# cschin/Peregrine

Hardware: AMD Instinct MI355X
Metric: confirmed overlaps/sec (ovlp_t records, index+overlap stages, seqdb resident in HBM) (higher is better)
Workload: dtype u8/u32 integer

## Files before the change

peregrine_amd/csrc/pgx_replay.h:

```cpp
#pragma once
#include "pgx_internal.h"

namespace pgx {
namespace rp {

constexpr uint32_t NIL = 0;
constexpr uint32_t NONE = 0xFFFFFFFFu;
constexpr int END_FUZZ = 48;
enum { T_OVERLAP = 0, T_CONTAINS = 1, T_CONTAINED = 2 };

constexpr uint32_t NIN = 58;
struct alignas(16) PHot {
  unsigned long long key;
  uint32_t own;
  uint32_t pad;
};
struct alignas(256) PCold {
  uint32_t cnt;
  uint32_t rhead;
  uint32_t in[NIN];
  uint32_t pad[4];
};
static_assert(sizeof(PHot) == 16 && sizeof(PCold) == 256, "pair slot = 16 hot bytes + four cold cache lines");
struct MSlot {
  unsigned long long a;
  uint32_t b;
  uint32_t req;
};
struct Item {
  uint32_t pslot;
  uint32_t info;
  uint32_t mslot;
  uint32_t next;
};
struct RNode {
  uint32_t next, bucket;
};
constexpr uint32_t I_GUESS = 1u << 18, I_UNFILED = 1u << 19;
#ifndef PGX_SPARSE_CAP
#define PGX_SPARSE_CAP 65536
#endif
constexpr uint32_t SPARSE_CAP = PGX_SPARSE_CAP;
constexpr uint32_t LIST_CAP = 262144;
constexpr uint32_t DEV_LIST = 0xFFFFFFFFu, DEV_LIST_WIN = 0xFFFFFFFEu;
enum : uint32_t { OV_ITEMS = 1, OV_NODES = 2, OV_REQS = 4, OV_PAIRS = 8, OV_MEMO = 16, OV_QOFF = 32, OV_PASSES = 64 };
constexpr uint8_t F_DUP = 1, F_GUESS = 2, F_UNFILED = 4;
constexpr uint8_t F_BIG = 8;

struct alignas(64) Counters {
  uint32_t item_top, rnode_top, nreq, overflow;
  uint32_t pad0[12];
  uint32_t ndirty, min_dirty, max_dirty, pad;
  uint32_t nbig;
  uint32_t nbig_total;
  uint32_t pad1[10];
  unsigned long long lookups, skips, evals, records;
#ifdef PGX_BIG_STATS
  uint32_t big_max_steps, big_long, big_long_n, big_evals;
  unsigned long long pad2[2];
#else
  unsigned long long pad2[4];
#endif
};

struct R {
  uint32_t nb;
  const uint32_t *bid, *bstart;
  const uint64_t *y0;
  const uint8_t *dir;
  const uint32_t *rlen;
  PHot *ph;
  PCold *pc;
  uint32_t cshift;
  uint32_t pmask;
  MSlot *mt;
  uint32_t mmask;
  Item *items;
  uint32_t item_cap;
  RNode *rn;
  uint32_t rn_cap;
  pgx_align_key *rq_key;
  pgx_match *rq_res;
  uint32_t req_cap, settled;
  uint32_t memo_used;
  uint8_t *dirty, *evaluated, *parity, *bflags, *ever;
  uint32_t *ihead, *inum, *ohead, *lookups, *skips;
  uint32_t *dlist;
  uint32_t *blist;
  uint32_t wlist0;
  uint4 *wcur;
  Counters *c;
  unsigned long long *spread;
  uint32_t bestn;
  uint32_t tail;
  int predict, predict2;
  uint32_t big_min;
  uint32_t dup_min;
  uint32_t wbig0;
};

__device__ __forceinline__ uint64_t mix64(uint64_t h) {
  h ^= h >> 33, h *= 0xff51afd7ed558ccdULL, h ^= h >> 33, h *= 0xc4ceb9fe1a85ec53ULL, h ^= h >> 33;
  return h;
}
__device__ __forceinline__ uint32_t own_enc(uint32_t j, uint32_t par, uint32_t type) { return ((j << 3) | (par << 2) | type) + 1; }
__device__ __forceinline__ uint32_t own_bucket(uint32_t v) { return (v - 1) >> 3; }
__device__ __forceinline__ uint32_t own_parity(uint32_t v) { return ((v - 1) >> 2) & 1; }
__device__ __forceinline__ uint32_t own_type(uint32_t v) { return (v - 1) & 3; }
__device__ __forceinline__ uint32_t lane_rank(uint64_t m) {
  return __builtin_amdgcn_mbcnt_hi((uint32_t)(m >> 32), __builtin_amdgcn_mbcnt_lo((uint32_t)m, 0u));
}
__device__ __forceinline__ long iabs64(long x) { return x < 0 ? -x : x; }

__device__ __forceinline__ bool classify(const pgx_match &m, uint32_t rlen0, uint32_t rlen1, uint32_t q_off, uint32_t *type) {
  const uint32_t slen0 = rlen0 - q_off, slen1 = rlen1;
  *type = T_OVERLAP;
  if (m.q_bgn < END_FUZZ && m.t_bgn < END_FUZZ &&
      (iabs64((long)slen0 - m.q_end) < END_FUZZ || iabs64((long)slen1 - m.t_end) < END_FUZZ) && m.q_end > 500 &&
      m.t_end > 500) {
    if (iabs64((long)rlen0 - ((long)m.q_end - m.q_bgn)) < END_FUZZ * 2 ||
        iabs64((long)rlen1 - ((long)m.t_end - m.t_bgn)) < END_FUZZ * 2)
      *type = rlen0 >= rlen1 ? T_CONTAINS : T_CONTAINED;
    return true;
  }
  return false;
}

__device__ __forceinline__ bool predict_contained(uint32_t rlen0, uint32_t rlen1, uint32_t q_off, int mq, int mt) {
  return (int)rlen1 - (int)(rlen0 - q_off) < mt || q_off < (uint32_t)mq;
}

__device__ __forceinline__ uint32_t pair_slot(const R &r, uint64_t pair) {
  const unsigned long long want = pair + 1;
  uint32_t i = (uint32_t)mix64(pair) & r.pmask;
  for (int probes = 0; probes < 1024; ++probes) {
    unsigned long long k = r.ph[i].key;
    if (k == want) return i;
    if (k == 0) {
      k = atomicCAS(&r.ph[i].key, 0ULL, want);
      if (k == 0 || k == want) return i;
    }
    i = (i + 1) & r.pmask;
  }
  atomicOr(&r.c->overflow, OV_PAIRS);
  return i;
}

__device__ __forceinline__ uint32_t pair_find(const R &r, uint64_t pair, uint32_t *own) {
  const unsigned long long want = pair + 1;
  uint32_t i = (uint32_t)mix64(pair) & r.pmask;
  for (int probes = 0; probes < 1024; ++probes) {
    const uint4 h = *reinterpret_cast<const uint4 *>(&r.ph[i]);
    const unsigned long long k = (unsigned long long)h.y << 32 | h.x;
    if (k == want) {
      *own = h.z;
      return i;
    }
    if (k == 0) break;
    i = (i + 1) & r.pmask;
  }
  *own = 0;
  return NONE;
}

__device__ __forceinline__ uint32_t memo_find(const R &r, unsigned long long a, uint32_t b, uint32_t *req) {
  uint32_t i = (uint32_t)mix64(a ^ mix64(b)) & r.mmask;
  for (int probes = 0; probes < 1024; ++probes) {
    const uint4 h = *reinterpret_cast<const uint4 *>(&r.mt[i]);
    const unsigned long long cur = (unsigned long long)h.y << 32 | h.x;
    if (cur == 0) break;
    if (cur == a && h.z == b + 1) {
      *req = h.w;
      return i;
    }
    i = (i + 1) & r.mmask;
  }
  *req = NONE;
  return NONE;
}

struct Ent {
  uint32_t rid, pos1;
};
__device__ __forceinline__ Ent entry_of(uint64_t y) { return Ent{(uint32_t)(y >> 32), (((uint32_t)y) >> 1) + 1}; }

constexpr uint32_t NCH = 256;
constexpr uint32_t SPREAD = 256;
constexpr uint32_t ICH = 128;

#ifndef PGX_REPLAY_GL
#define PGX_REPLAY_GL 16
#endif
constexpr int GL = PGX_REPLAY_GL;
constexpr uint32_t GPW = 64 / GL, GPB = 256 / GL;
__device__ __forceinline__ uint64_t gbits(uint64_t wave_mask, int gbase) { return (wave_mask >> gbase) & ((1ULL << GL) - 1ULL); }

__device__ __forceinline__ uint64_t bucket_of_group(const R &r, uint32_t lo, uint32_t hi, uint32_t nlist, uint32_t g) {
  if (nlist) {
    const uint32_t n = nlist == DEV_LIST ? min(r.c->ndirty, SPARSE_CAP) : nlist == DEV_LIST_WIN ? min(r.c->ndirty, LIST_CAP) : nlist;
    return g < n ? (uint64_t)r.dlist[g] : (uint64_t)hi;
  }
  return (uint64_t)lo + g;
}

__device__ __forceinline__ void mark_readers(const R &r, uint32_t slot, uint32_t j) {
  const uint32_t *w = reinterpret_cast<const uint32_t *>(&r.pc[slot >> r.cshift]);
  const uint4 h1 = *reinterpret_cast<const uint4 *>(w);
  const uint32_t c = min(h1.x, NIN);
  if (c > 0 && h1.z > j + 1 && h1.z <= r.nb) r.dirty[h1.z - 1] = 1;
  if (c > 1 && h1.w > j + 1 && h1.w <= r.nb) r.dirty[h1.w - 1] = 1;
  for (uint32_t q = 2; q < c; q += 8) {
    const uint4 a = *reinterpret_cast<const uint4 *>(w + 2 + q), b = *reinterpret_cast<const uint4 *>(w + 6 + q);
    const uint32_t x[8] = {a.x, a.y, a.z, a.w, b.x, b.y, b.z, b.w};
#pragma unroll
    for (uint32_t k = 0; k < 8; ++k)
      if (q + k < c && x[k] > j + 1 && x[k] <= r.nb) r.dirty[x[k] - 1] = 1;
  }
  if (c < NIN) return;
  for (uint32_t nd = h1.y; nd != NIL; nd = r.rn[nd - 1].next) {
    const uint32_t rb = r.rn[nd - 1].bucket;
    if (rb > j) r.dirty[rb] = 1;
  }
}

struct M128 {
  uint64_t lo, hi;
};
__device__ __forceinline__ int popc128(M128 m) { return __popcll(m.lo) + __popcll(m.hi); }
__device__ __forceinline__ bool any128(M128 m) { return (m.lo | m.hi) != 0; }
__device__ __forceinline__ int ctz128(M128 m) { return m.lo ? __builtin_ctzll(m.lo) : 64 + __builtin_ctzll(m.hi); }
__device__ __forceinline__ int nth128(M128 m, uint32_t nth) {
  const uint32_t cl = (uint32_t)__popcll(m.lo);
  uint64_t w = m.lo;
  int base = 0;
  if (nth > cl) w = m.hi, nth -= cl, base = 64;
  for (uint32_t k = 1; k < nth; ++k) w &= w - 1;
  return base + __builtin_ctzll(w);
}
__device__ __forceinline__ M128 upto128(int stop) {
  M128 m;
  m.lo = stop >= 63 ? ~0ULL : ((2ULL << stop) - 1ULL);
  m.hi = stop < 64 ? 0ULL : (stop >= 127 ? ~0ULL : ((2ULL << (stop - 64)) - 1ULL));
  return m;
}
__device__ __forceinline__ M128 and128(M128 a, M128 b) { return M128{a.lo & b.lo, a.hi & b.hi}; }
__device__ __forceinline__ M128 andn128(M128 a, M128 b) { return M128{a.lo & ~b.lo, a.hi & ~b.hi}; }
__device__ __forceinline__ M128 shr128(M128 m, uint32_t s) {
  if (s >= 128) return M128{0, 0};
  if (s >= 64) return M128{m.hi >> (s - 64), 0};
  if (s == 0) return m;
  return M128{m.lo >> s | m.hi << (64 - s), m.hi >> s};
}




#ifndef PGX_BIG_NW
#define PGX_BIG_NW 8
#endif
constexpr int BIG_NW = PGX_BIG_NW;
constexpr int BIG_NR = BIG_NW / 2;
constexpr uint32_t BIG_WG = 512;
constexpr uint32_t SET_CAP = 2048, CLAIM_CAP = 1024;
constexpr uint32_t CB = 4096;

__global__ void k_setup(R r, uint32_t *hist);
__global__ void k_init_slots(uint4 *__restrict__ wcur, uint32_t nslots, uint32_t n_dense, uint32_t wlist0, Counters *c);
__global__ void k_eval(R r, uint32_t lo, uint32_t hi, uint32_t nlist);
template <int GLT, int PW>
__global__ void k_eval_rows(R r, uint32_t lo, uint32_t hi, uint32_t nlist);
__global__ void k_eval_big(R r, uint32_t lo, uint32_t hi, uint32_t nlist);
__global__ void k_update(R r, uint32_t lo, uint32_t hi, uint32_t nlist);
__global__ void k_count_a(R r, uint32_t rlo, uint32_t rhi, uint32_t *__restrict__ blk);
__global__ void k_count_b(R r, uint32_t rlo, uint32_t rhi, const uint32_t *__restrict__ blk, uint32_t nblk);
__global__ void k_file(R r, uint32_t limit);
__global__ void k_settle(R r);
__global__ void k_emit(R r, const uint32_t *__restrict__ off, pgx_ovlp *__restrict__ out);
__global__ void k_count_pairs(const PHot *__restrict__ ph, uint32_t cap, unsigned long long *__restrict__ out);

}
}
```

peregrine_amd/csrc/pgx_replay.hip:

```cpp
#include <optional>

#include "pgx_replay.h"

namespace pgx {
using namespace rp;
namespace {
uint32_t pow2_at_least(size_t x) {
  size_t c = 1024;
  while (c < x) c <<= 1;
  return (uint32_t)c;
}
unsigned cdiv256(size_t n) { return (unsigned)((n + 255) / 256); }
int env_int(const char *name, int unset) { return getenv(name) ? atoi(getenv(name)) : unset; }
template <typename T>
void alloc_tagged(const char *tag, DevBuf<T> &buf, size_t n) { MemTag t(tag); buf.alloc(n); }

constexpr size_t ITEMS_PER_ENTRY = 6, ITEMS_PER_BUCKET = 64, NODES_PER_ENTRY = 8, REQS_PER_ENTRY = 1;
constexpr size_t STATE_PER_BUCKET = 64;
constexpr double TABLE_LOAD = 0.4;

struct Usage {
  double pairs = 0, reqs = 0, items = 0, nodes = 0;
  void raise(const Usage &u) { pairs = std::max(pairs, u.pairs), reqs = std::max(reqs, u.reqs), items = std::max(items, u.items), nodes = std::max(nodes, u.nodes); }
};
struct Mult {
  double items = 1, nodes = 1, reqs = 1, pairs = 1, memo = 1;
  static Mult from(const Usage &learned, size_t ne, size_t nb) {
    Mult m;
    if (learned.pairs > 0) {
      const double items_default = (double)ITEMS_PER_ENTRY + (double)ITEMS_PER_BUCKET * (double)nb / ne;
      m.items = std::max(0.2, learned.items * 1.25 / items_default), m.nodes = std::max(0.02, learned.nodes * 2 / NODES_PER_ENTRY);
      m.reqs = std::max(1.0, learned.reqs * 1.2);
      m.pairs = std::max(1.0, learned.pairs / TABLE_LOAD), m.memo = std::max(1.0, learned.reqs / TABLE_LOAD);
    }
    if (getenv("PGX_REPLAY_PAIRS_X")) m.pairs = atof(getenv("PGX_REPLAY_PAIRS_X"));
    if (getenv("PGX_REPLAY_MEMO_X")) m.memo = atof(getenv("PGX_REPLAY_MEMO_X"));
    return m;
  }
  void grow(uint32_t ov) {
    auto arena = [](double &m) { m = m < 1 ? 1.0 : m * 2; };
    if (ov & OV_ITEMS) arena(items);
    if (ov & OV_NODES) arena(nodes);
    if (ov & OV_REQS) arena(reqs);
    if (ov & OV_PAIRS) pairs *= 4;
    if (ov & (OV_MEMO | OV_REQS)) memo *= 4;
  }
};

struct Sizes {
  uint32_t pcap, mcap;
  uint32_t cshift = 0;
  size_t ccap = 0;
  uint32_t item_cap, rn_cap, req_cap;
  Sizes(size_t ne, size_t nb, const Mult &m) {
    const size_t top = 0x7FFFFFF0u;
    pcap = pow2_at_least((size_t)(ne * m.pairs)), mcap = pow2_at_least((size_t)(ne * m.memo));
    item_cap = (uint32_t)std::min((size_t)((ne * ITEMS_PER_ENTRY + nb * ITEMS_PER_BUCKET) * m.items) +
                                      (size_t)(nb / GPW + 2 + SPARSE_CAP + 8 + BIG_WG * BIG_NW) * ICH + (1u << 20), top);
    rn_cap = (uint32_t)std::min((size_t)(ne * NODES_PER_ENTRY * m.nodes) + (1u << 20), top);
    req_cap = (uint32_t)std::min((size_t)(ne * REQS_PER_ENTRY * m.reqs) + 65536, top);
  }
  void share_readers(size_t free_bytes) {
    if (getenv("PGX_REPLAY_COLD_SHIFT")) cshift = (uint32_t)std::min(3, std::max(0, env_int("PGX_REPLAY_COLD_SHIFT", 0)));
    else
      while (cshift < 3 && ((size_t)pcap >> cshift) * sizeof(PCold) > free_bytes / 3) ++cshift;
    ccap = ((size_t)pcap >> cshift) + 1;
  }
};
size_t default_need(size_t ne, size_t nb) {
  return (size_t)pow2_at_least(ne) * (sizeof(PHot) + sizeof(PCold) + sizeof(MSlot)) +
         ne * (ITEMS_PER_ENTRY * sizeof(Item) + NODES_PER_ENTRY * sizeof(RNode) + REQS_PER_ENTRY * (sizeof(pgx_align_key) + sizeof(pgx_match))) +
         nb * (ITEMS_PER_BUCKET * sizeof(Item) + STATE_PER_BUCKET) + (256u << 20);
}

struct Tables {
  DevBuf<PHot> hot;
  DevBuf<PCold> cold;
  DevBuf<MSlot> memo;
  bool hot_zero = false, cold_zero = false, memo_zero = false;
  bool held() const { return hot.p != nullptr; }
  size_t bytes() const { return hot.n * sizeof(PHot) + cold.n * sizeof(PCold) + memo.n * sizeof(MSlot); }
  void alloc(size_t pcap, size_t ccap, size_t mcap) {
    if (pcap && hot.n != pcap) alloc_tagged("replay.pair_table_hot", hot, pcap), hot_zero = false;
    if (ccap && cold.n != ccap) alloc_tagged("replay.pair_table_readers", cold, ccap), cold_zero = false;
    if (mcap && memo.n != mcap) alloc_tagged("replay.memo_table", memo, mcap), memo_zero = false;
  }
  void clear(hipStream_t s) {
    if (!hot_zero) PGX_HIP(hipMemsetAsync(hot.p, 0, hot.n * sizeof(PHot), s));
    if (!cold_zero) PGX_HIP(hipMemsetAsync(cold.p, 0, cold.n * sizeof(PCold), s));
    if (!memo_zero) PGX_HIP(hipMemsetAsync(memo.p, 0, memo.n * sizeof(MSlot), s));
    hot_zero = cold_zero = memo_zero = true;
  }
  void drop() { hot.release(), cold.release(), memo.release(), hot_zero = cold_zero = memo_zero = false; }
};
}

struct ReplayState {
  Tables pre;
  size_t last_pcap = 0, last_ccap = 0, last_mcap = 0;
  Usage learned;
  void forget() { pre.drop(), last_pcap = last_ccap = last_mcap = 0, learned = Usage(); }
  Counters *hc = nullptr;
  unsigned long long *hs = nullptr;
  hipStream_t side_stream = nullptr;
  hipEvent_t side_ev[2] = {nullptr, nullptr};
  void handles() {
    if (!hc) PGX_HIP(hipHostMalloc((void **)&hc, sizeof(Counters), hipHostMallocDefault));
    if (!hs) PGX_HIP(hipHostMalloc((void **)&hs, SPREAD * 8 * sizeof(unsigned long long), hipHostMallocDefault));
    if (!side_stream) PGX_HIP(hipStreamCreateWithFlags(&side_stream, hipStreamNonBlocking));
    for (auto &e : side_ev)
      if (!e) PGX_HIP(hipEventCreateWithFlags(&e, hipEventDisableTiming));
  }
  ~ReplayState() {
    if (hc) (void)hipHostFree(hc);
    if (hs) (void)hipHostFree(hs);
    if (side_stream) (void)hipStreamDestroy(side_stream);
    for (auto &e : side_ev)
      if (e) (void)hipEventDestroy(e);
  }
};
void CacheFree::operator()(ReplayState *r) const { delete r; }

namespace {
constexpr size_t WIN0 = 16384, WIN1 = 131072;
constexpr size_t DENSE_DEN = 3;
constexpr size_t TAIL_MAX = 4000;
constexpr uint32_t AHEAD = 24;
constexpr int CHAIN = 8;
constexpr size_t BIG_BATCH = 100000;

enum class Narrow { eval, rows };
struct Walk {
  const pgx_seqdb *const db;
  ReplayState &rs;
  const size_t nb, ne;
  const int band;
  const bool trace;
  const hipStream_t s = ctx().stream;
  const double t0 = wall_ms();
  const bool timed = env_int("PGX_REPLAY_TIMING", 0) != 0;
  const bool deep = env_int("PGX_TRACE", 0) >= 2;
  const size_t window = getenv("PGX_REPLAY_WIN") ? (size_t)atoll(getenv("PGX_REPLAY_WIN")) : (size_t)262144;
  const int inner = env_int("PGX_REPLAY_K", 2);
  Sizes z;
  Tables tab;
  DevBuf<uint32_t> bid, words, dlist, blist, cblk;
  DevBuf<Item> items;
  DevBuf<RNode> rn;
  DevBuf<pgx_align_key> rq_key;
  DevBuf<pgx_match> rq_res;
  DevBuf<uint8_t> bytes;
  DevBuf<uint4> wcur;
  DevBuf<Counters> dc;
  DevBuf<unsigned long long> spread;
  R r;
  Counters *hc = nullptr;
  bool use_big = false;
  size_t n_dirty;
  uint32_t d_lo = 0, d_hi;
  bool known = true;
  bool have_list = false;
  unsigned sweeps = 0, rounds_total = 0;
  size_t first_req = 0;
  size_t first_batch = 0;
  double align_ms = 0;
  Walk(const pgx_seqdb *db_, size_t nb_, size_t ne_, int band_, bool trace_, const Mult &mult)
      : db(db_), rs(get_or_make(db_->caches.replay)), nb(nb_), ne(ne_), band(band_), trace(trace_), z(ne_, nb_, mult), n_dirty(nb_), d_hi((uint32_t)nb_) {
    memset(&r, 0, sizeof(r));
  }
  void alloc_tables() {
    Tables &pre = rs.pre;
    const bool forced = getenv("PGX_REPLAY_COLD_SHIFT") != nullptr;
    const size_t pre_hold = pre.bytes();
    const bool take = pre.held() && pre.hot.n == z.pcap && pre.memo.n == z.mcap && !forced;
    if (take) tab.hot = std::move(pre.hot), tab.memo = std::move(pre.memo), tab.hot_zero = tab.memo_zero = true;
    tab.alloc(z.pcap, 0, 0);
    size_t free_b = 0, total_b = 0;
    const bool measured = !forced && hipMemGetInfo(&free_b, &total_b) == hipSuccess;
    z.share_readers(measured ? free_b + dev_cache_free_bytes() + pre_hold : SIZE_MAX);
    if (take && pre.cold.n == z.ccap) tab.cold = std::move(pre.cold), tab.cold_zero = true;
    else pre.cold.release();
    tab.alloc(z.pcap, z.ccap, z.mcap);
    pre.drop();
    r.ph = tab.hot.p, r.pc = tab.cold.p, r.cshift = z.cshift, r.pmask = z.pcap - 1, r.mt = tab.memo.p, r.mmask = z.mcap - 1;
  }
  void alloc_state() {
    r.item_cap = z.item_cap, r.rn_cap = z.rn_cap, r.req_cap = z.req_cap;
    alloc_tagged("replay.items", items, r.item_cap), alloc_tagged("replay.reader_nodes", rn, r.rn_cap);
    alloc_tagged("replay.requests", rq_key, r.req_cap), alloc_tagged("replay.requests", rq_res, r.req_cap);
    r.items = items.p, r.rn = rn.p, r.rq_key = rq_key.p, r.rq_res = rq_res.p;
    bytes.alloc(nb * 5), words.alloc(nb * 5);
    r.dirty = bytes.p, r.evaluated = bytes.p + nb, r.parity = bytes.p + 2 * nb, r.bflags = bytes.p + 3 * nb, r.ever = bytes.p + 4 * nb;
    r.ihead = words.p, r.inum = words.p + nb, r.ohead = words.p + 2 * nb, r.lookups = words.p + 3 * nb, r.skips = words.p + 4 * nb;
    wcur.alloc(nb + 2 + SPARSE_CAP + 1 + (size_t)BIG_WG * BIG_NW);
    r.wcur = wcur.p, r.wlist0 = (uint32_t)(nb + 2), r.wbig0 = (uint32_t)(nb + 2 + SPARSE_CAP + 1);
    dlist.alloc(LIST_CAP), blist.alloc(LIST_CAP + 64), dc.alloc(1), spread.alloc(SPREAD * 8);
    r.dlist = dlist.p, r.blist = blist.p, r.c = dc.p, r.spread = spread.p;
  }
  void setup(const DevicePairs &dp, const uint32_t *visit_bids, const uint32_t *d_bids, uint32_t bestn) {
    rs.handles(), hc = rs.hc;
    r.nb = (uint32_t)nb;
    if (!d_bids) bid.alloc(nb), bid.upload(visit_bids, nb);
    r.bid = d_bids ? d_bids : bid.p, r.bstart = dp.bstart.p, r.y0 = dp.y0.p, r.dir = dp.dir.p, r.rlen = db->d_rlen.p;
    alloc_tables();
    alloc_state();
    r.big_min = (uint32_t)std::max(0, env_int("PGX_REPLAY_BIG", 48));
    r.dup_min = (uint32_t)std::max(0, env_int("PGX_REPLAY_DUP", 12));
    r.predict = std::max(END_FUZZ * 2 - 8, 1), r.predict2 = END_FUZZ * 2 - 8;
    r.bestn = bestn, r.settled = 0;
    PGX_HIP(hipMemsetAsync(spread.p, 0, SPREAD * 8 * sizeof(unsigned long long), s));
    {
      std::optional<KernelTimer> tm;
      if (timed) tm.emplace("replay_misc", nb);
      const bool took = tab.hot_zero, took_cold = tab.cold_zero;
      tab.clear(s);
      if (trace && took) fprintf(stderr, "[pgx]   replay tables taken over pre-cleared (pair table%s, memo)\n", took_cold ? ", reader lists" : "");
      PGX_HIP(hipMemsetAsync(bytes.p, 0, nb * 5, s));
      PGX_HIP(hipMemsetAsync(words.p, 0, nb * 5 * sizeof(uint32_t), s));
      PGX_HIP(hipMemsetAsync(dc.p, 0, sizeof(Counters), s));
      hipLaunchKernelGGL(k_init_slots, dim3(cdiv256(wcur.n)), dim3(256), 0, s, wcur.p, (uint32_t)wcur.n, (uint32_t)(nb / GPW + 2), r.wlist0, dc.p);
      if (trace) setup_with_histogram();
      else hipLaunchKernelGGL(k_setup, dim3(cdiv256(nb)), dim3(256), 0, s, r, (uint32_t *)nullptr);
    }
    if (r.big_min || r.dup_min) {
      fetch(false);
      use_big = hc->nbig_total != 0;
    }
    cblk.alloc((nb + CB - 1) / CB * 3);
  }
  void setup_with_histogram() {
    DevBuf<uint32_t> hist(32);
    PGX_HIP(hipMemsetAsync(hist.p, 0, 32 * sizeof(uint32_t), s));
    hipLaunchKernelGGL(k_setup, dim3(cdiv256(nb)), dim3(256), 0, s, r, hist.p);
    uint32_t h[32];
    hist.download(h, 32);
    sync();
    fprintf(stderr, "[pgx]   buckets by entries / 8 (last class: >= 120):");
    for (int i = 0; i < 16; ++i) fprintf(stderr, " %u", h[i]);
    fprintf(stderr, "\n[pgx]   ... of those holding a read twice (one partner at a time):");
    for (int i = 0; i < 16; ++i) fprintf(stderr, " %u", h[16 + i]);
    fprintf(stderr, "\n");
  }
  void fetch(bool totals, bool counters = true) {
    if (counters) PGX_HIP(hipMemcpyAsync(hc, dc.p, sizeof(Counters), hipMemcpyDeviceToHost, s));
    if (totals) PGX_HIP(hipMemcpyAsync(rs.hs, spread.p, SPREAD * 8 * sizeof(unsigned long long), hipMemcpyDeviceToHost, s));
    sync();
    if (totals) sum_totals();
  }
  void sum_totals() {
    const unsigned long long *hs = rs.hs;
    hc->evals = hc->lookups = hc->skips = 0;
    hc->records = 0;
    for (uint32_t i = 0; i < SPREAD; ++i) hc->evals += hs[i * 8], hc->lookups += hs[i * 8 + 1], hc->skips += hs[i * 8 + 2], hc->records += hs[i * 8 + 7];
#ifdef PGX_BIG_STATS
    unsigned long long b3 = 0, b4 = 0, b5 = 0, b6 = 0, b7 = 0;
    for (uint32_t i = 0; i < SPREAD; ++i) b3 += hs[i * 8 + 3], b4 += hs[i * 8 + 4], b5 += hs[i * 8 + 5], b6 += hs[i * 8 + 6], b7 += hs[i * 8 + 7];
    fprintf(stderr, "[pgx]   k_eval_big so far: %u evaluations, %llu steps, %llu rows committed; steps cut at a duplicate %llu, ended by a containment %llu, all rows %llu; longest %u steps, %u evaluations of >= 64 steps (entries %u)\n",
            hc->big_evals, b3, b4, b5, b6, b7, hc->big_max_steps, hc->big_long, hc->big_long_n);
#endif
#ifdef PGX_SETTLE_STATS
    unsigned long long c3 = 0, c4 = 0, c5 = 0, c6 = 0;
    for (uint32_t i = 0; i < SPREAD; ++i) c3 += hs[i * 8 + 3], c4 += hs[i * 8 + 4], c5 += hs[i * 8 + 5], c6 += hs[i * 8 + 6];
    fprintf(stderr, "[pgx]   wrong guesses so far: type %llu, rejected short overlap %llu, rejected no match %llu, rejected other %llu\n", c3, c4, c5, c6);
#endif
  }
  void learn_dirty() { n_dirty = hc->ndirty, known = true, d_lo = n_dirty ? hc->min_dirty : 0, d_hi = n_dirty ? hc->max_dirty + 1 : 0; }
  uint32_t gave_up(uint32_t ov) {
    if (trace || !(ov & (OV_ITEMS | OV_NODES | OV_REQS | OV_PAIRS | OV_MEMO)))
      fprintf(stderr, "[pgx] note: the device replay gave up (code %u: items %u of %u, reader nodes %u of %u, requests %u of %u)\n", ov,
              hc->item_top, r.item_cap, hc->rnode_top, r.rn_cap, hc->nreq, r.req_cap);
    return ov;
  }
  void count(uint32_t lo = 0, uint32_t hi = NONE) {
    hi = std::min<uint32_t>(hi, (uint32_t)nb);
    const uint32_t nbl = std::max<uint32_t>(1, (hi - lo + CB - 1) / CB);
    std::optional<KernelTimer> tm;
    if (timed) tm.emplace("replay_misc", 0);
    hipLaunchKernelGGL(k_count_a, dim3(nbl), dim3(256), 0, s, r, lo, hi, cblk.p);
    hipLaunchKernelGGL(k_count_b, dim3(nbl), dim3(256), 0, s, r, lo, hi, cblk.p, nbl);
  }
  void count_all() { count(), have_list = true; }
  void pass(uint32_t lo, uint32_t hi, uint32_t list, Narrow narrow, uint32_t groups, uint64_t units) {
    std::optional<KernelTimer> tm;
    if (timed) tm.emplace(narrow == Narrow::rows ? "replay_rows" : "replay_dense", units);
    const bool walled = deep && list != DEV_LIST;
    double td = 0, t_eval = 0;
    if (walled) sync(), td = wall_ms();
    if (list == DEV_LIST_WIN) count(lo, hi);
    const uint32_t a = list ? 0u : lo, b = list ? (uint32_t)nb : hi;
    const uint32_t big_a = list == DEV_LIST_WIN ? LIST_CAP : list == DEV_LIST ? groups : lo;
    const dim3 big_grid(std::min<uint32_t>(BIG_WG, groups)), big_block(64 * BIG_NW), grid(cdiv256((size_t)groups * GL));
    const bool side = use_big && list && !timed && !deep;
    if (side) {
      PGX_HIP(hipEventRecord(rs.side_ev[0], s));
      PGX_HIP(hipStreamWaitEvent(rs.side_stream, rs.side_ev[0], 0));
      hipLaunchKernelGGL(k_eval_big, big_grid, big_block, 0, rs.side_stream, r, big_a, b, list);
      PGX_HIP(hipEventRecord(rs.side_ev[1], rs.side_stream));
    }
    if (narrow == Narrow::rows) hipLaunchKernelGGL((k_eval_rows<64, 16>), dim3(cdiv256((size_t)groups * 64)), dim3(256), 0, s, r, a, b, list);
    else hipLaunchKernelGGL(k_eval, grid, dim3(256), 0, s, r, a, b, list);
    tm.reset();
    if (side) {
      PGX_HIP(hipStreamWaitEvent(s, rs.side_ev[1], 0));
    } else if (use_big) {
      if (timed) tm.emplace("replay_big", 0);
      hipLaunchKernelGGL(k_eval_big, big_grid, big_block, 0, s, r, big_a, b, list);
      tm.reset();
    }
    if (walled) sync(), t_eval = wall_ms() - td, td = wall_ms();
    if (timed) tm.emplace("replay_update", 0);
    hipLaunchKernelGGL(k_update, grid, dim3(256), 0, s, r, a, b, list);
    tm.reset();
    if (walled) sync(), fprintf(stderr, "[pgx]     iteration: eval %.3f ms, update %.3f ms\n", t_eval, wall_ms() - td);
  }
  void dense_round(bool first_pass) {
    const size_t a_lo = d_lo & ~(size_t)63;
    const size_t win = n_dirty > window / 4 ? window : (size_t)(d_hi - a_lo);
    const size_t cap = first_pass ? std::min(WIN1, win) : win;
    size_t step = first_pass ? std::min(WIN0, cap) : win;
    for (size_t lo = a_lo, nxt; lo < d_hi; lo = nxt, step = std::min(step * 2, cap)) {
      nxt = lo + step;
      const uint32_t hi = (uint32_t)std::min<size_t>(d_hi, nxt), n = hi - (uint32_t)lo;
      for (int k = 0; k < inner; ++k) {
        const bool from_list = !(first_pass && k == 0) && n <= LIST_CAP;
        pass((uint32_t)lo, hi, from_list ? DEV_LIST_WIN : 0u, Narrow::eval, n, k == 0 ? n : 0);
      }
    }
    count_all();
  }
  void sparse_chain() {
    if (!have_list) count_all();
    const size_t est = known && n_dirty <= SPARSE_CAP / 4 ? std::max<size_t>(n_dirty * 4, 1024) : (size_t)SPARSE_CAP;
    const uint32_t groups = (uint32_t)std::min<size_t>(est, SPARSE_CAP);
    for (int c = 0; c < CHAIN; ++c) {
      pass(0, (uint32_t)nb, DEV_LIST, Narrow::rows, groups, 0);
      count_all();
    }
  }
  uint32_t file_and_fetch(unsigned rounds) {
    {
      std::optional<KernelTimer> tm;
      if (timed) tm.emplace("replay_misc", 0);
      hipLaunchKernelGGL(k_file, dim3(cdiv256(nb)), dim3(256), 0, s, r, (uint32_t)nb);
    }
    fetch(trace);
    if (hc->overflow) return hc->overflow;
    learn_dirty();
    r.memo_used = hc->nreq != 0;
    if (trace)
      fprintf(stderr, "[pgx]   round %u: %zu dirty left in [%u, %u), %llu evaluations, t = +%.2f ms\n", rounds, n_dirty, d_lo, d_hi,
              (unsigned long long)hc->evals, wall_ms() - t0);
    return 0;
  }
  uint32_t align_and_settle(size_t nreq) {
    const double a0 = wall_ms();
    const size_t batch = nreq - first_req;
    if (sweeps == 1) first_batch = batch;
    r.tail = batch <= std::max(TAIL_MAX, first_batch / 256) ? AHEAD : 0u;
    dev_align(db, r.rq_key + first_req, batch, band, r.rq_res + first_req, sweeps > 2 ? 2 : sweeps > 1 ? 1 : 0);
    r.settled = (uint32_t)nreq, first_req = nreq;
    {
      std::optional<KernelTimer> tm;
      if (timed) tm.emplace("replay_misc", 0);
      hipLaunchKernelGGL(k_settle, dim3(cdiv256(nb)), dim3(256), 0, s, r);
    }
    count_all();
    if (batch > BIG_BATCH) {
      fetch(false);
      if (hc->overflow) return hc->overflow;
      learn_dirty();
      if (trace) fprintf(stderr, "[pgx]   alignments + settle %.2f ms, %zu buckets guessed wrong\n", wall_ms() - a0, n_dirty);
    } else {
      known = false;
      n_dirty = std::min<size_t>(batch, SPARSE_CAP / 8);
      if (trace) fprintf(stderr, "[pgx]   %zu alignments + settle enqueued in %.2f ms\n", batch, wall_ms() - a0);
    }
    align_ms += wall_ms() - a0;
    return 0;
  }
  uint32_t emit(const std::function<pgx_ovlp *(size_t)> &alloc_out, RecordSink *sink, size_t *n_out, pgx_overlap_stats *st, Usage *usage) {
    const double e0 = wall_ms();
    DevBuf<uint32_t> off(nb + 1);
    exclusive_sum(r.inum, off.p, nb);
    uint32_t last_off = 0, last_num = 0;
    PGX_HIP(hipMemcpyAsync(&last_off, off.p + nb - 1, 4, hipMemcpyDeviceToHost, s));
    PGX_HIP(hipMemcpyAsync(&last_num, r.inum + nb - 1, 4, hipMemcpyDeviceToHost, s));
    fetch(false);
    if (hc->overflow) return hc->overflow;
    const size_t nrec = (size_t)last_off + last_num;
    DevBuf<unsigned long long> d_keys(1);
    PGX_HIP(hipMemsetAsync(d_keys.p, 0, sizeof(unsigned long long), s));
    hipLaunchKernelGGL(k_count_pairs, dim3((unsigned)std::min<size_t>(cdiv256(z.pcap), 4096)), dim3(256), 0, s, tab.hot.p, z.pcap, d_keys.p);
    results_wait();
    pgx_ovlp *host = alloc_out(nrec);
    DevBuf<pgx_ovlp> d_out;
    alloc_tagged("replay.records_out", d_out, std::max<size_t>(nrec, 1));
    {
      std::optional<KernelTimer> tm;
      if (timed) tm.emplace("replay_emit", nrec);
      hipLaunchKernelGGL(k_emit, dim3(cdiv256(nb)), dim3(256), 0, s, r, off.p, d_out.p);
      if (nrec && sink) sink->take(std::move(d_out), nrec);
      else if (nrec && results_async() && !timed) results_copy_async(host, std::move(d_out), nrec);
      else if (nrec) PGX_HIP(hipMemcpyAsync(host, d_out.p, nrec * sizeof(pgx_ovlp), hipMemcpyDeviceToHost, s));
    }
    unsigned long long n_keys = 0;
    d_keys.download(&n_keys, 1);
    fetch(true, false);
    usage->pairs = (double)n_keys / ne, usage->reqs = (double)hc->nreq / ne, usage->items = (double)hc->item_top / ne, usage->nodes = (double)hc->rnode_top / ne;
    if (trace)
      fprintf(stderr, "[pgx]   tables: %llu read pairs in %u slots (load %.2f), %u alignments in %u memo slots (load %.2f), items %u of %u, reader nodes %u of %u, requests %u of %u\n",
              n_keys, z.pcap, (double)n_keys / z.pcap, hc->nreq, z.mcap, (double)hc->nreq / z.mcap, hc->item_top, r.item_cap, hc->rnode_top, r.rn_cap, hc->nreq, r.req_cap);
    rs.last_pcap = z.pcap, rs.last_mcap = z.mcap, rs.last_ccap = z.ccap;
    *n_out = nrec;
    if (st) {
      st->n_align_needed = hc->lookups, st->n_seen_skip = hc->skips, st->n_align_gpu = first_req, st->rounds = sweeps, st->n_evaluations = hc->evals;
#if !defined(PGX_BIG_STATS) && !defined(PGX_SETTLE_STATS)
      st->stream_checksum = hc->records;
#endif
    }
    if (trace)
      fprintf(stderr, "[pgx] device replay: %u sweeps, %u rounds, %llu evaluations, %zu records; emit %.2f ms; alignments %.2f ms; total %.2f ms\n",
              sweeps, rounds_total, (unsigned long long)hc->evals, nrec, wall_ms() - e0, align_ms, wall_ms() - t0);
    return 0;
  }
  uint32_t run(const std::function<pgx_ovlp *(size_t)> &alloc_out, RecordSink *sink, size_t *n_out, pgx_overlap_stats *st, Usage *usage) {
    for (;;) {
      ++sweeps;
      const double p0 = wall_ms();
      unsigned rounds = 0;
      do {
        ++rounds;
        if (known && n_dirty * DENSE_DEN > nb) dense_round(sweeps == 1 && rounds == 1);
        sparse_chain();
        if (const uint32_t ov = file_and_fetch(rounds)) return gave_up(ov);
        if (n_dirty && rounds > 20000) return gave_up(OV_PASSES);
      } while (n_dirty);
      rounds_total += rounds;
      const size_t nreq = hc->nreq;
      if (trace)
        fprintf(stderr, "[pgx] device sweep %u: %u rounds, %llu evaluations so far, %.2f ms, %zu requests\n", sweeps, rounds,
                (unsigned long long)hc->evals, wall_ms() - p0, nreq - first_req);
      if (nreq == first_req) break;
      if (const uint32_t ov = align_and_settle(nreq)) return gave_up(ov);
      if (!n_dirty) break;
    }
    const uint32_t ov = emit(alloc_out, sink, n_out, st, usage);
    return ov ? gave_up(ov) : 0;
  }
};

__global__ void k_place_bids(const uint32_t *__restrict__ ids_all, const uint32_t *__restrict__ psrc, const uint32_t *__restrict__ pcnt,
                             const uint64_t *__restrict__ pdst, uint32_t n_groups, uint32_t *__restrict__ bid) {
  const uint32_t i = blockIdx.x * blockDim.x + threadIdx.x;
  if (i >= n_groups) return;
  const uint32_t src = psrc[i], n = pcnt[i];
  const uint64_t dst = pdst[i];
  for (uint32_t k = 0; k < n; ++k) bid[dst + k] = ids_all[src + k];
}
}
void dev_place_bids(const uint32_t *ids_all, size_t n_ids, const uint32_t *psrc, const uint32_t *pcnt, const uint64_t *pdst,
                    size_t n_groups, size_t nb, DevBuf<uint32_t> &bid) {
  bid.alloc(std::max<size_t>(nb, 1));
  if (!n_groups || !nb) return;
  DevBuf<uint32_t> d_ids(n_ids), d_src(n_groups), d_cnt(n_groups);
  DevBuf<uint64_t> d_dst(n_groups);
  d_ids.upload(ids_all, n_ids), d_src.upload(psrc, n_groups), d_cnt.upload(pcnt, n_groups), d_dst.upload(pdst, n_groups);
  hipLaunchKernelGGL(k_place_bids, dim3((unsigned)((n_groups + 255) / 256)), dim3(256), 0, ctx().stream, d_ids.p, d_src.p, d_cnt.p, d_dst.p,
                     (uint32_t)n_groups, bid.p);
  sync();
}

void replay_drop_precleared(const pgx_seqdb *db) {
  if (db->caches.replay) db->caches.replay->pre.drop();
}

void replay_preclear(const pgx_seqdb *db) {
  ReplayState &rs = get_or_make(db->caches.replay);
  Tables &pre = rs.pre;
  if (!rs.last_pcap || pre.held() || env_int("PGX_REPLAY_PRECLEAR", 1) == 0) return;
  size_t free_b = 0, total_b = 0;
  const size_t need = rs.last_pcap * sizeof(PHot) + rs.last_ccap * sizeof(PCold) + rs.last_mcap * sizeof(MSlot);
  if (hipMemGetInfo(&free_b, &total_b) != hipSuccess || need > free_b + dev_cache_free_bytes()) return;
  try {
    pre.alloc(rs.last_pcap, rs.last_ccap, rs.last_mcap);
    pre.clear(ctx().stream);
  } catch (const Fail &) {
    (void)hipGetLastError();
    pre.drop();
  }
}

bool dev_replay(const pgx_seqdb *db, const DevicePairs &dp, const uint32_t *visit_bids, const uint32_t *d_bids, size_t nb, size_t n_entries,
                uint32_t bestn, int band, uint32_t ovlp_upper, const std::function<pgx_ovlp *(size_t)> &alloc_out, RecordSink *sink,
                size_t *n_out, pgx_overlap_stats *st, bool trace) {
  *n_out = 0;
  ReplayState &rs = get_or_make(db->caches.replay);
  struct DropPre {
    Tables &pre;
    ~DropPre() { pre.drop(); }
  } drop_pre{rs.pre};
  if (ovlp_upper > 128 || nb >= (1u << 29) - 2 || n_entries >= (1ULL << 31) || !dp.valid) return false;
  if (nb == 0) {
    alloc_out(0);
    return true;
  }
  const size_t ne = std::max<size_t>(n_entries, 1024);
  {
    const size_t need = default_need(ne, nb);
    size_t free_b = 0, total_b = 0;
    if (hipMemGetInfo(&free_b, &total_b) == hipSuccess && need > free_b) {
      rs.pre.drop();
      dev_cache_trim();
      if (hipMemGetInfo(&free_b, &total_b) != hipSuccess || need > free_b) {
        fprintf(stderr, "[pgx] note: the device replay's tables (%.1f GB) do not fit the free device memory (%.1f GB); the host replay takes over\n",
                need / 1e9, free_b / 1e9);
        return false;
      }
    }
  }
  Mult mult = Mult::from(rs.learned, ne, nb);
  for (int attempt = 0; attempt < 4; ++attempt) {
    Usage usage;
    uint32_t ov;
    try {
      MemTag mem_tag("replay.other");
      Walk w(db, nb, ne, band, trace, mult);
      w.setup(dp, visit_bids, d_bids, bestn);
      ov = w.run(alloc_out, sink, n_out, st, &usage);
    } catch (const Fail &f) {
      if (f.code != PGX_ENOMEM && !(f.code == PGX_EHIP && strstr(pgx_last_error(), "hipMalloc"))) throw;
      (void)hipGetLastError();
      const bool had_learned = rs.learned.pairs > 0;
      rs.forget();
      dev_cache_trim();
      if (!had_learned || attempt > 0) {
        fprintf(stderr, "[pgx] note: the device replay's tables could not be allocated (%s); the host replay takes over\n", pgx_last_error());
        return false;
      }
      mult = Mult();
      if (trace) fprintf(stderr, "[pgx]   the tables sized by the last stage's use do not fit (%s): once more with the default sizes\n", pgx_last_error());
      continue;
    }
    if (!ov) {
      rs.learned.raise(usage);
      if (st) st->replay_attempts = (uint32_t)attempt + 1;
      return true;
    }
    if (ov & (OV_QOFF | OV_PASSES)) break;
    mult.grow(ov);
    if (trace) fprintf(stderr, "[pgx]   next attempt with items x %g, reader nodes x %g, requests x %g, pair table x %g, memo table x %g\n", mult.items, mult.nodes, mult.reqs, mult.pairs, mult.memo);
  }
  fprintf(stderr, "[pgx] note: the device replay's tables overflowed; the host replay takes over\n");
  return false;
}

}
```

peregrine_amd/csrc/pgx_replay_eval.hip:

```cpp
#include "pgx_replay.h"

namespace pgx {
namespace rp {

__global__ __launch_bounds__(256) void k_eval(R r, uint32_t lo, uint32_t hi, uint32_t nlist) {
  __shared__ uint32_t s_rid[GPB][128], s_pos[GPB][128], s_rl[GPB][128];
  __shared__ uint8_t s_dir[GPB][128];
  const int lane = threadIdx.x & 63, gl = lane & (GL - 1), gbase = lane & ~(GL - 1), gib = threadIdx.x / GL;
  const uint32_t wave = (blockIdx.x * blockDim.x + threadIdx.x) >> 6;
  const uint64_t jj = bucket_of_group(r, lo, hi, nlist, wave * GPW + (uint32_t)(lane / GL));
  const uint32_t j = (uint32_t)jj;
  bool alive = jj < hi && r.dirty[j] && !r.c->overflow;
  if (alive && (r.bflags[j] & F_BIG)) {
    if (gl == 0) {
      const uint32_t at = atomicAdd(&r.c->nbig, 1u);
      if (at < LIST_CAP) r.blist[at] = j;
    }
    alive = false;
  }
  {
    const uint64_t am = __ballot(alive);
    if (!am) return;
    if (lane == (int)__builtin_ctzll(am)) atomicAdd(&r.spread[(wave % SPREAD) * 8], (unsigned long long)(__popcll(am) / GL));
  }
  const uint32_t wave_id = nlist ? r.wlist0 + wave : (uint32_t)(((uint64_t)lo + (uint64_t)wave * GPW) / GPW);
  const uint4 wc = r.wcur[wave_id];
  uint32_t rcur = wc.x, rend = wc.y;
  uint32_t icur = wc.z, iend = wc.w;
  uint32_t s0 = 0, n = 0;
  bool dup = false, first_eval = true;
  if (alive) {
    const uint32_t b = r.bid[j];
    s0 = r.bstart[b], n = r.bstart[b + 1] - s0;
    dup = (r.bflags[j] & F_DUP) != 0;
    first_eval = r.ever[j] == 0;
    for (uint32_t i = (uint32_t)gl; i < n; i += GL) {
      const uint64_t y = r.y0[s0 + i];
      const uint32_t rid = (uint32_t)(y >> 32);
      s_rid[gib][i] = rid, s_pos[gib][i] = (((uint32_t)y) >> 1) + 1, s_dir[gib][i] = r.dir[s0 + i], s_rl[gib][i] = r.rlen[rid];
    }
    if (gl == 0) {
      r.dirty[j] = 0;
      r.evaluated[j] = 1;
      r.ever[j] = 1;
      r.parity[j] ^= 1;
      r.ohead[j] = r.ihead[j];
    }
  }
  uint64_t clo = 0, chi = 0;
  auto cget = [&](uint32_t i) { return (((i < 64 ? clo : chi) >> (i & 63)) & 1) != 0; };
  uint32_t head = NIL, num = 0, lookups = 0, skips = 0;
  uint32_t chunk = 0;
  bool any_guess = false, any_unfiled = false;
  int ai = (int)n - 1;
  bool row_open = false;
  uint32_t pbase = 0, got = 0, rid0 = 0, pos0 = 0, rlen0 = 0, dir0 = 0;
  bool p_reg = false;
  uint32_t p_idx = 0, p_slot = 0;
  auto resolve_pending = [&]() -> bool {
    if (p_reg && p_idx < NIN) r.pc[p_slot >> r.cshift].in[p_idx] = j + 1, p_reg = false;
    const uint64_t rm = __ballot(p_reg);
    if (rm) {
      const uint32_t total = (uint32_t)__popcll(rm);
      if (rcur + total > rend) {
        uint32_t base = 0;
        if (lane == 0) base = atomicAdd(&r.c->rnode_top, NCH);
        base = (uint32_t)__shfl((int)base, 0, 64);
        if ((uint64_t)base + NCH > r.rn_cap) {
          atomicOr(&r.c->overflow, OV_NODES);
          return false;
        }
        rcur = base, rend = base + NCH;
      }
      if (p_reg) {
        const uint32_t node = rcur + lane_rank(rm);
        const uint32_t old = atomicExch(&r.pc[p_slot >> r.cshift].rhead, node + 1);
        r.rn[node] = RNode{old, j};
      }
      rcur += total;
      p_reg = false;
    }
    return true;
  };
  for (;;) {
    if (alive && !row_open) {
      do --ai;
      while (ai >= 0 && cget((uint32_t)ai));
      if (ai < 0 || r.bestn == 0) {
        if (gl == 0) {
          r.ihead[j] = head, r.inum[j] = num, r.lookups[j] = lookups, r.skips[j] = skips;
          r.bflags[j] = (uint8_t)((dup ? F_DUP : 0) | (any_guess ? F_GUESS : 0) | (any_unfiled ? F_UNFILED : 0));
        }
        alive = false;
      } else {
        rid0 = s_rid[gib][ai], pos0 = s_pos[gib][ai], rlen0 = s_rl[gib][ai], dir0 = s_dir[gib][ai];
        got = 0, pbase = (uint32_t)ai + 1, row_open = true;
      }
    }
    if (!__ballot(alive)) {
      if (!resolve_pending()) return;
      if (lane == 0) r.wcur[wave_id] = make_uint4(rcur, rend, icur, iend);
      break;
    }
    const uint32_t step = dup ? 1u : (uint32_t)GL;
    const uint32_t pi = pbase + (uint32_t)gl;
    bool valid = alive && (uint32_t)gl < step && pi < n && !cget(pi);
    uint32_t rid1 = 0, pos1 = 0;
    if (valid) {
      rid1 = s_rid[gib][pi], pos1 = s_pos[gib][pi];
      if (rid1 == rid0) valid = false;
    }
    uint32_t slot = NONE, v = 0;
    const uint64_t pair = rid0 < rid1 ? ((uint64_t)rid0 << 32 | rid1) : ((uint64_t)rid1 << 32 | rid0);
    if (valid) slot = pair_find(r, pair, &v);
    const uint64_t vm = __ballot(valid);
    bool present = false, accepted = false, guessed = false;
    uint32_t ptype = 0, type = 0, mslot = NONE;
    if (valid) {
      present = v != 0 && own_bucket(v) < j;
      ptype = present ? own_type(v) : 0;
      if (!present && dup && slot != NONE)
        for (uint32_t it = head; it != NIL; it = r.items[it - 1].next)
          if (r.items[it - 1].pslot == slot) {
            present = true, ptype = (r.items[it - 1].info >> 16) & 3;
            break;
          }
      if (!present) {
        const uint32_t rlen1 = s_rl[gib][pi], dir1 = s_dir[gib][pi];
        const uint32_t q_off = pos0 - pos1;
        if (q_off >= (1u << 30)) atomicOr(&r.c->overflow, OV_QOFF);
        uint32_t req = NONE;
        if (r.memo_used) mslot = memo_find(r, (unsigned long long)rid0 << 32 | rid1, q_off << 2 | dir0 << 1 | dir1, &req);
        if (req < r.settled) {
          accepted = classify(r.rq_res[req], rlen0, rlen1, q_off, &type);
        } else {
          accepted = true, guessed = true, type = T_OVERLAP;
          if (r.predict && predict_contained(rlen0, rlen1, q_off, r.predict, r.predict2)) type = rlen0 >= rlen1 ? T_CONTAINS : T_CONTAINED;
        }
      }
    }
    if (!resolve_pending()) return;
    const uint64_t Vg = gbits(vm, gbase);
    const uint64_t P = gbits(__ballot(valid && present), gbase);
    const uint64_t PO = gbits(__ballot(valid && present && ptype == T_OVERLAP), gbase);
    const uint64_t A = gbits(__ballot(valid && !present && accepted), gbase);
    const uint64_t AO = gbits(__ballot(valid && !present && accepted && type == T_OVERLAP), gbase);
    const uint64_t AC = gbits(__ballot(valid && !present && accepted && type == T_CONTAINED), gbase);
    uint64_t AP = gbits(__ballot(valid && !present && accepted && type == T_CONTAINS), gbase);
    const uint64_t inc = PO | AO;
    int stop = GL;
    if (alive && row_open) {
      const uint32_t need = r.bestn - got;
      if ((uint32_t)__popcll(inc) >= need) {
        uint64_t m = inc;
        for (uint32_t k = 1; k < need; ++k) m &= m - 1;
        stop = __builtin_ctzll(m);
      }
      if (AC) stop = min(stop, (int)__builtin_ctzll(AC));
    }
    const uint64_t proc = (2ULL << stop) - 1ULL;
    const uint64_t ins = A & proc;
    {
      bool reg = valid && ((proc >> gl) & 1);
      if (reg && slot == NONE) slot = pair_slot(r, pair);
      if (reg && !first_eval) {
        const uint32_t *w = reinterpret_cast<const uint32_t *>(&r.pc[slot >> r.cshift]);
        const uint4 h1 = *reinterpret_cast<const uint4 *>(w);
        const uint32_t c = min(h1.x, NIN);
        if ((c > 0 && h1.z == j + 1) || (c > 1 && h1.w == j + 1)) reg = false;
        for (uint32_t q = 2; q < c && reg; q += 8) {
          const uint4 a = *reinterpret_cast<const uint4 *>(w + 2 + q), b = *reinterpret_cast<const uint4 *>(w + 6 + q);
          const uint32_t x[8] = {a.x, a.y, a.z, a.w, b.x, b.y, b.z, b.w};
#pragma unroll
          for (uint32_t k = 0; k < 8; ++k)
            if (q + k < c && x[k] == j + 1) reg = false;
        }
      }
      if (reg) p_idx = atomicAdd(&r.pc[slot >> r.cshift].cnt, 1u), p_slot = slot, p_reg = true;
    }
    const bool my_ins = valid && !present && accepted && ((proc >> gl) & 1);
    const uint32_t cins = (uint32_t)__popcll(ins);
    const bool need_chunk = cins != 0 && (num == 0 || ((num + cins - 1) >> 4) != ((num - 1) >> 4));
    uint32_t fresh = 0;
    {
      const uint64_t cm = __ballot(need_chunk && gl == 0);
      if (cm) {
        const uint32_t want = 16u * (uint32_t)__popcll(cm);
        if (icur + want > iend) {
          const uint32_t take = want > ICH ? want : ICH;
          uint32_t base = 0;
          if (lane == (int)__builtin_ctzll(cm)) base = atomicAdd(&r.c->item_top, take);
          base = (uint32_t)__shfl((int)base, (int)__builtin_ctzll(cm), 64);
          if ((uint64_t)base + take > r.item_cap) {
            atomicOr(&r.c->overflow, OV_ITEMS);
            return;
          }
          icur = base, iend = base + take;
        }
        fresh = icur + 16u * (uint32_t)__popcll(cm & ((1ULL << gbase) - 1ULL));
        icur += want;
      }
    }
    if (cins) {
      if (my_ins) {
        const uint32_t ord = num + (uint32_t)__popcll(ins & ((1ULL << gl) - 1ULL));
        const bool in_fresh = need_chunk && (num == 0 || (ord >> 4) != ((num - 1) >> 4));
        const uint32_t idx = (in_fresh ? fresh : chunk) + (ord & 15);
        uint32_t next;
        if (ord == 0) next = NIL;
        else if ((ord & 15) == 0) next = chunk + 16;
        else next = idx;
        uint32_t info = (uint32_t)ai | pi << 8 | type << 16;
        if (guessed) info |= I_GUESS;
        if (mslot == NONE) info |= I_UNFILED;
        r.items[idx] = Item{slot, info, mslot, next};
      }
      const uint32_t last = num + cins - 1;
      if (need_chunk && (num == 0 || (last >> 4) != ((num - 1) >> 4))) chunk = fresh;
      head = chunk + (last & 15) + 1;
      num += cins;
    }
    {
      const uint64_t g1 = gbits(__ballot(my_ins && guessed), gbase), g2 = gbits(__ballot(my_ins && mslot == NONE), gbase);
      any_guess |= g1 != 0, any_unfiled |= g2 != 0;
    }
    if (alive && row_open) {
      got += (uint32_t)__popcll(inc & proc);
      skips += (uint32_t)__popcll(P & proc);
      lookups += (uint32_t)__popcll(Vg & ~P & proc);
      AP &= proc;
      if (AP) {
        if (pbase < 64) {
          clo |= AP << pbase;
          if (pbase) chi |= AP >> (64 - pbase);
        } else {
          chi |= AP << (pbase - 64);
        }
      }
      if (AC & proc) {
        if (ai < 64) clo |= 1ULL << ai;
        else chi |= 1ULL << (ai - 64);
      }
      if (stop < GL || pbase + step >= n) row_open = false;
      else pbase += step;
    }
  }
}

template <int GLT, int PW>
__global__ __launch_bounds__(256) void k_eval_rows(R r, uint32_t lo, uint32_t hi, uint32_t nlist) {
  constexpr uint32_t GPWT = 64 / GLT, GPBT = 256 / GLT;
  constexpr int SH = PW == 16 ? 4 : 2;
  constexpr uint64_t RM = (1ULL << PW) - 1ULL;
  __shared__ uint32_t s_rid[GPBT][128], s_pos[GPBT][128], s_rl[GPBT][128];
  __shared__ uint8_t s_dir[GPBT][128];
  const int lane = threadIdx.x & 63, gl = lane & (GLT - 1), gbase = lane & ~(GLT - 1), gib = threadIdx.x / GLT;
  const uint32_t wave = (blockIdx.x * blockDim.x + threadIdx.x) >> 6;
  const uint64_t jj = bucket_of_group(r, lo, hi, nlist, wave * GPWT + (uint32_t)(lane / GLT));
  const uint32_t j = (uint32_t)jj;
  bool alive = jj < hi && r.dirty[j] && !r.c->overflow;
  if (alive && (r.bflags[j] & F_BIG)) {
    if (gl == 0) {
      const uint32_t at = atomicAdd(&r.c->nbig, 1u);
      if (at < LIST_CAP) r.blist[at] = j;
    }
    alive = false;
  }
  {
    const uint64_t am = __ballot(alive);
    if (!am) return;
    if (lane == (int)__builtin_ctzll(am)) atomicAdd(&r.spread[(wave % SPREAD) * 8], (unsigned long long)(__popcll(am) / GLT));
  }
  const uint32_t wave_id = nlist ? r.wlist0 + wave : (uint32_t)(((uint64_t)lo + (uint64_t)wave * GPWT) / GPWT);
  const uint4 wc = r.wcur[wave_id];
  uint32_t rcur = wc.x, rend = wc.y;
  uint32_t icur = wc.z, iend = wc.w;
  uint32_t s0 = 0, n = 0;
  bool dup = false, first_eval = true;
  if (alive) {
    const uint32_t b = r.bid[j];
    s0 = r.bstart[b], n = r.bstart[b + 1] - s0;
    dup = (r.bflags[j] & F_DUP) != 0;
    first_eval = r.ever[j] == 0;
    for (uint32_t i = (uint32_t)gl; i < n; i += GLT) {
      const uint64_t y = r.y0[s0 + i];
      const uint32_t rid = (uint32_t)(y >> 32);
      s_rid[gib][i] = rid, s_pos[gib][i] = (((uint32_t)y) >> 1) + 1, s_dir[gib][i] = r.dir[s0 + i], s_rl[gib][i] = r.rlen[rid];
    }
    if (gl == 0) {
      r.dirty[j] = 0;
      r.evaluated[j] = 1;
      r.ever[j] = 1;
      r.parity[j] ^= 1;
      r.ohead[j] = r.ihead[j];
    }
  }
  auto gbits = [&](uint64_t wave_mask, int) { return GLT == 64 ? wave_mask : ((wave_mask >> gbase) & ((1ULL << (GLT & 63)) - 1ULL)); };
  uint64_t clo = 0, chi = 0;
  auto cget = [&](uint32_t i) { return (((i < 64 ? clo : chi) >> (i & 63)) & 1) != 0; };
  auto cset = [&](uint32_t i) {
    if (i < 64) clo |= 1ULL << i;
    else chi |= 1ULL << (i - 64);
  };
  uint32_t head = NIL, num = 0, lookups = 0, skips = 0;
  uint32_t chunk = 0;
  bool any_guess = false, any_unfiled = false;
  int done_to = (int)n - 1;
  bool row_open = false;
  int cur_row = 0, a0 = -1, a1 = -1, a2 = -1, a3 = -1, nrows = 0;
  uint32_t pbase = 0, got = 0;
  bool p_reg = false;
  uint32_t p_idx = 0, p_slot = 0;
  auto resolve_pending = [&]() -> bool {
    if (p_reg && p_idx < NIN) r.pc[p_slot >> r.cshift].in[p_idx] = j + 1, p_reg = false;
    const uint64_t rm = __ballot(p_reg);
    if (rm) {
      const uint32_t total = (uint32_t)__popcll(rm);
      if (rcur + total > rend) {
        uint32_t base = 0;
        if (lane == 0) base = atomicAdd(&r.c->rnode_top, NCH);
        base = (uint32_t)__shfl((int)base, 0, 64);
        if ((uint64_t)base + NCH > r.rn_cap) {
          atomicOr(&r.c->overflow, OV_NODES);
          return false;
        }
        rcur = base, rend = base + NCH;
      }
      if (p_reg) {
        const uint32_t node = rcur + lane_rank(rm);
        const uint32_t old = atomicExch(&r.pc[p_slot >> r.cshift].rhead, node + 1);
        r.rn[node] = RNode{old, j};
      }
      rcur += total;
      p_reg = false;
    }
    return true;
  };
  for (;;) {
    if (alive && !row_open) {
      nrows = 0, a0 = a1 = a2 = a3 = -1;
      int x = done_to;
      while (nrows < 4) {
        do --x;
        while (x >= 0 && cget((uint32_t)x));
        if (x < 0) break;
        if (nrows == 0) a0 = x;
        else if (nrows == 1) a1 = x;
        else if (nrows == 2) a2 = x;
        else a3 = x;
        ++nrows;
      }
      if (nrows == 0 || r.bestn == 0) {
        if (gl == 0) {
          r.ihead[j] = head, r.inum[j] = num, r.lookups[j] = lookups, r.skips[j] = skips;
          r.bflags[j] = (uint8_t)((dup ? F_DUP : 0) | (any_guess ? F_GUESS : 0) | (any_unfiled ? F_UNFILED : 0));
        }
        alive = false;
      } else if (dup) {
        cur_row = a0, got = 0, pbase = (uint32_t)a0 + 1, row_open = true;
      }
    }
    if (!__ballot(alive)) {
      if (!resolve_pending()) return;
      if (lane == 0) r.wcur[wave_id] = make_uint4(rcur, rend, icur, iend);
      break;
    }
    const bool single = row_open;
    const uint32_t step = dup ? 1u : (uint32_t)GLT;
    const int q = gl >> SH;
    const int myrow = single ? cur_row : (q == 0 ? a0 : q == 1 ? a1 : q == 2 ? a2 : a3);
    const uint32_t pi = single ? pbase + (uint32_t)gl : (uint32_t)(myrow + 1 + (gl & (PW - 1)));
    bool valid = alive && (single ? (uint32_t)gl < step : q < nrows) && pi < n && !cget(pi);
    uint32_t rid0 = 0, pos0 = 0, rlen0 = 0, dir0 = 0, rid1 = 0, pos1 = 0;
    if (valid) {
      rid0 = s_rid[gib][myrow], pos0 = s_pos[gib][myrow], rlen0 = s_rl[gib][myrow], dir0 = s_dir[gib][myrow];
      rid1 = s_rid[gib][pi], pos1 = s_pos[gib][pi];
      if (rid1 == rid0) valid = false;
    }
    uint32_t slot = NONE, v = 0;
    const uint64_t pair = rid0 < rid1 ? ((uint64_t)rid0 << 32 | rid1) : ((uint64_t)rid1 << 32 | rid0);
    if (valid) slot = pair_find(r, pair, &v);
    const uint64_t vm = __ballot(valid);
    bool present = false, accepted = false, guessed = false;
    uint32_t ptype = 0, type = 0, mslot = NONE;
    if (valid) {
      present = v != 0 && own_bucket(v) < j;
      ptype = present ? own_type(v) : 0;
      if (!present && dup && slot != NONE)
        for (uint32_t it = head; it != NIL; it = r.items[it - 1].next)
          if (r.items[it - 1].pslot == slot) {
            present = true, ptype = (r.items[it - 1].info >> 16) & 3;
            break;
          }
      if (!present) {
        const uint32_t rlen1 = s_rl[gib][pi], dir1 = s_dir[gib][pi];
        const uint32_t q_off = pos0 - pos1;
        if (q_off >= (1u << 30)) atomicOr(&r.c->overflow, OV_QOFF);
        uint32_t req = NONE;
        if (r.memo_used) mslot = memo_find(r, (unsigned long long)rid0 << 32 | rid1, q_off << 2 | dir0 << 1 | dir1, &req);
        if (req < r.settled) {
          accepted = classify(r.rq_res[req], rlen0, rlen1, q_off, &type);
        } else {
          accepted = true, guessed = true, type = T_OVERLAP;
          if (r.predict && predict_contained(rlen0, rlen1, q_off, r.predict, r.predict2)) type = rlen0 >= rlen1 ? T_CONTAINS : T_CONTAINED;
        }
      }
    }
    if (!resolve_pending()) return;
    const uint64_t Vg = gbits(vm, gbase);
    const uint64_t P = gbits(__ballot(valid && present), gbase);
    const uint64_t PO = gbits(__ballot(valid && present && ptype == T_OVERLAP), gbase);
    const uint64_t A = gbits(__ballot(valid && !present && accepted), gbase);
    const uint64_t AO = gbits(__ballot(valid && !present && accepted && type == T_OVERLAP), gbase);
    const uint64_t AC = gbits(__ballot(valid && !present && accepted && type == T_CONTAINED), gbase);
    const uint64_t AP = gbits(__ballot(valid && !present && accepted && type == T_CONTAINS), gbase);
    const uint64_t inc = PO | AO;
    uint64_t proc = 0;
    if (alive && single) {
      int stop = GLT;
      const uint32_t need = r.bestn - got;
      if ((uint32_t)__popcll(inc) >= need) {
        uint64_t m = inc;
        for (uint32_t k = 1; k < need; ++k) m &= m - 1;
        stop = __builtin_ctzll(m);
      }
      if (AC) stop = min(stop, (int)__builtin_ctzll(AC));
      proc = stop >= 63 ? ~0ULL : ((2ULL << stop) - 1ULL);
      got += (uint32_t)__popcll(inc & proc);
      for (uint64_t m = AP & proc; m; m &= m - 1) cset(pbase + (uint32_t)__builtin_ctzll(m));
      if (AC & proc) cset((uint32_t)cur_row);
      if (stop < GLT || pbase + step >= n) row_open = false, done_to = cur_row;
      else pbase += step;
    } else if (alive) {
      int committed = 0;
#pragma unroll
      for (int k = 0; k < 4; ++k) {
        if (k >= nrows || committed != k) continue;
        const int row = k == 0 ? a0 : k == 1 ? a1 : k == 2 ? a2 : a3;
        const uint32_t gone = (uint32_t)shr128(M128{clo, chi}, (uint32_t)row + 1).lo & (uint32_t)RM;
        const uint32_t inc_k = (uint32_t)((inc >> (PW * k)) & RM) & ~gone, ac_k = (uint32_t)((AC >> (PW * k)) & RM) & ~gone,
                       ap_k = (uint32_t)((AP >> (PW * k)) & RM) & ~gone;
        int stop = PW;
        if ((uint32_t)__popc(inc_k) >= r.bestn) {
          uint32_t m = inc_k;
          for (uint32_t t = 1; t < r.bestn; ++t) m &= m - 1;
          stop = __builtin_ctz(m);
        }
        if (ac_k) stop = min(stop, (int)__builtin_ctz(ac_k));
        if (stop == PW && (uint32_t)row + 1 + PW < n) continue;
        const uint32_t proc_k = (stop < PW ? (2u << stop) - 1u : (uint32_t)RM) & ~gone;
        proc |= (uint64_t)proc_k << (PW * k);
        ++committed;
        for (uint32_t m = ap_k & proc_k; m; m &= m - 1) cset((uint32_t)row + 1 + (uint32_t)__builtin_ctz(m));
        if (ac_k & proc_k) cset((uint32_t)row);
      }
      if (committed == 0) cur_row = a0, got = 0, pbase = (uint32_t)a0 + 1, row_open = true;
      else done_to = committed == 1 ? a0 : committed == 2 ? a1 : committed == 3 ? a2 : a3;
    }
    skips += (uint32_t)__popcll(P & proc);
    lookups += (uint32_t)__popcll(Vg & ~P & proc);
    const uint64_t ins = A & proc;
    {
      bool reg = valid && ((proc >> gl) & 1);
      if (reg && slot == NONE) slot = pair_slot(r, pair);
      if (reg && !first_eval) {
        const uint32_t *w = reinterpret_cast<const uint32_t *>(&r.pc[slot >> r.cshift]);
        const uint4 h1 = *reinterpret_cast<const uint4 *>(w);
        const uint32_t c = min(h1.x, NIN);
        if ((c > 0 && h1.z == j + 1) || (c > 1 && h1.w == j + 1)) reg = false;
        for (uint32_t qq = 2; qq < c && reg; qq += 8) {
          const uint4 a = *reinterpret_cast<const uint4 *>(w + 2 + qq), b = *reinterpret_cast<const uint4 *>(w + 6 + qq);
          const uint32_t x[8] = {a.x, a.y, a.z, a.w, b.x, b.y, b.z, b.w};
#pragma unroll
          for (uint32_t k = 0; k < 8; ++k)
            if (qq + k < c && x[k] == j + 1) reg = false;
        }
      }
      if (reg) p_idx = atomicAdd(&r.pc[slot >> r.cshift].cnt, 1u), p_slot = slot, p_reg = true;
    }
    const bool my_ins = valid && !present && accepted && ((proc >> gl) & 1);
    const uint32_t cins = (uint32_t)__popcll(ins);
    static_assert(GLT == 64, "one bucket per wavefront: the chunk allocation below is wave-uniform");
    if (cins) {
      const uint32_t cur_no = num ? (num - 1) >> 4 : 0;
      const uint32_t first_new = num ? cur_no + 1 : 0;
      const uint32_t last = num + cins - 1, last_no = last >> 4;
      const uint32_t nnew = last_no + 1 > first_new ? last_no + 1 - first_new : 0;
      uint32_t fresh = 0;
      if (nnew) {
        const uint32_t want = 16u * nnew;
        if (icur + want > iend) {
          const uint32_t take = want > ICH ? want : ICH;
          uint32_t base = 0;
          if (lane == 0) base = atomicAdd(&r.c->item_top, take);
          base = (uint32_t)__shfl((int)base, 0, 64);
          if ((uint64_t)base + take > r.item_cap) {
            atomicOr(&r.c->overflow, OV_ITEMS);
            return;
          }
          icur = base, iend = base + take;
        }
        fresh = icur, icur += want;
      }
      auto base_of = [&](uint32_t no) { return no >= first_new ? fresh + 16u * (no - first_new) : chunk; };
      if (my_ins) {
        const uint32_t ord = num + (uint32_t)__popcll(ins & ((1ULL << gl) - 1ULL));
        const uint32_t idx = base_of(ord >> 4) + (ord & 15);
        uint32_t next;
        if (ord == 0) next = NIL;
        else if ((ord & 15) == 0) next = base_of((ord >> 4) - 1) + 16;
        else next = idx;
        uint32_t info = (uint32_t)myrow | pi << 8 | type << 16;
        if (guessed) info |= I_GUESS;
        if (mslot == NONE) info |= I_UNFILED;
        r.items[idx] = Item{slot, info, mslot, next};
      }
      chunk = base_of(last_no);
      head = chunk + (last & 15) + 1;
      num += cins;
    }
    {
      const uint64_t g1 = gbits(__ballot(my_ins && guessed), gbase), g2 = gbits(__ballot(my_ins && mslot == NONE), gbase);
      any_guess |= g1 != 0, any_unfiled |= g2 != 0;
    }
  }
}
template __global__ void k_eval_rows<64, 16>(R r, uint32_t lo, uint32_t hi, uint32_t nlist);

__global__ __launch_bounds__(64 * BIG_NW) void k_eval_big(R r, uint32_t lo, uint32_t hi, uint32_t nlist) {
  enum { MV = 0, MP, MPO, MA, MAO, MAC, MAP, MGU, MUF, MDF, NM };
  __shared__ uint32_t s_rid[128], s_pos[128], s_rl[128];
  __shared__ uint8_t s_dir[128];
  __shared__ uint64_t s_m[BIG_NW][NM];
  __shared__ uint32_t s_fresh, s_abort, s_bail;
  __shared__ unsigned long long s_setk[SET_CAP];
  __shared__ uint8_t s_sett[SET_CAP];
  __shared__ unsigned long long s_clk[CLAIM_CAP];
  __shared__ uint32_t s_clw[CLAIM_CAP];
  const int lane = threadIdx.x & 63, w = threadIdx.x >> 6;
  const uint32_t wave_id = r.wbig0 + blockIdx.x * BIG_NW + (uint32_t)w;
  const uint4 wc = r.wcur[wave_id];
  uint32_t rcur = wc.x, rend = wc.y;
  uint32_t icur = wc.z, iend = wc.w;
  if (threadIdx.x == 0) s_abort = 0;
  const uint32_t list_limit = nlist ? lo : 0u;
  const uint32_t nbig = min(r.c->nbig, LIST_CAP);
  for (uint32_t g = blockIdx.x; g < nbig; g += gridDim.x) {
  {
    const uint32_t e = r.blist[g];
    if ((e & 0x80000000u) && (e & 0x7FFFFFFFu) >= list_limit) continue;
    const uint32_t j = (e & 0x80000000u) ? (r.dlist[e & 0x7FFFFFFFu] & 0x7FFFFFFFu) : e;
    __syncthreads();
    if (threadIdx.x == 0) {
      if (r.c->overflow) s_abort = 1;
      s_bail = 0, s_fresh = (j < hi && r.dirty[j]) ? 1u : 0u;
    }
    __syncthreads();
    if (s_abort) break;
    if (!s_fresh) continue;
    const uint32_t b = r.bid[j], s0 = r.bstart[b], n = r.bstart[b + 1] - s0;
    const bool first_eval = r.ever[j] == 0;
    const bool dup = (r.bflags[j] & F_DUP) != 0;
    for (uint32_t i = threadIdx.x; i < n; i += blockDim.x) {
      const uint64_t y = r.y0[s0 + i];
      const uint32_t rid = (uint32_t)(y >> 32);
      s_rid[i] = rid, s_pos[i] = (((uint32_t)y) >> 1) + 1, s_dir[i] = r.dir[s0 + i], s_rl[i] = r.rlen[rid];
    }
    if (dup) {
      for (uint32_t i = threadIdx.x; i < SET_CAP; i += blockDim.x) s_setk[i] = 0;
      for (uint32_t i = threadIdx.x; i < CLAIM_CAP; i += blockDim.x) s_clk[i] = 0, s_clw[i] = 0xFFFFFFFFu;
    }
    __syncthreads();
    if (threadIdx.x == 0) {
      r.dirty[j] = 0, r.evaluated[j] = 1, r.ever[j] = 1, r.parity[j] ^= 1, r.ohead[j] = r.ihead[j];
      atomicAdd(&r.spread[(blockIdx.x % SPREAD) * 8], 1ULL);
    }
    uint64_t clo = 0, chi = 0;
    auto cget = [&](uint32_t i) { return (((i < 64 ? clo : chi) >> (i & 63)) & 1) != 0; };
    auto cset = [&](uint32_t i) {
      if (i < 64) clo |= 1ULL << i;
      else chi |= 1ULL << (i - 64);
    };
    uint32_t head = NIL, num = 0, lookups = 0, skips = 0, chunk = 0;
    bool any_guess = false, any_unfiled = false;
    int done_to = (int)n - 1;
    bool row_open = false;
    int cur_row = 0;
    uint32_t pbase = 0, got = 0;
    bool p_reg = false;
    uint32_t p_idx = 0, p_slot = 0;
    auto resolve_pending = [&]() {
      if (p_reg && p_idx < NIN) r.pc[p_slot >> r.cshift].in[p_idx] = j + 1, p_reg = false;
      const uint64_t rm = __ballot(p_reg);
      if (rm) {
        const uint32_t total = (uint32_t)__popcll(rm);
        if (rcur + total > rend) {
          uint32_t base = 0;
          if (lane == 0) base = atomicAdd(&r.c->rnode_top, NCH);
          base = (uint32_t)__shfl((int)base, 0, 64);
          if ((uint64_t)base + NCH > r.rn_cap) {
            atomicOr(&r.c->overflow, OV_NODES);
            s_abort = 1;
            p_reg = false;
            return;
          }
          rcur = base, rend = base + NCH;
        }
        if (p_reg) {
          const uint32_t node = rcur + lane_rank(rm);
          const uint32_t old = atomicExch(&r.pc[p_slot >> r.cshift].rhead, node + 1);
          r.rn[node] = RNode{old, j};
        }
        rcur += total;
        p_reg = false;
      }
    };
#ifdef PGX_BIG_STATS
    uint32_t st_steps = 0, st_rows = 0, st_cut = 0, st_cont = 0, st_full = 0;
#endif
    for (;;) {
      int a[BIG_NR], nrows = 0;
#pragma unroll
      for (int k = 0; k < BIG_NR; ++k) a[k] = -1;
      if (row_open) {
        a[0] = cur_row, nrows = 1;
      } else {
        for (int x = done_to; nrows < BIG_NR;) {
          do --x;
          while (x >= 0 && cget((uint32_t)x));
          if (x < 0) break;
          a[nrows++] = x;
        }
      }
      if (nrows == 0 || r.bestn == 0) break;
      const int q = w >> 1, off = (w & 1) * 64 + lane;
      const int myrow = a[q];
      const uint32_t first = row_open ? pbase : (uint32_t)(myrow + 1);
      const uint32_t pi = first + (uint32_t)off;
      const uint32_t wi = (uint32_t)(q * 128 + off);
      bool valid = q < nrows && pi < n && !cget(pi);
      uint32_t rid0 = 0, pos0 = 0, rlen0 = 0, dir0 = 0, rid1 = 0, pos1 = 0;
      if (valid) {
        rid0 = s_rid[myrow], pos0 = s_pos[myrow], rlen0 = s_rl[myrow], dir0 = s_dir[myrow];
        rid1 = s_rid[pi], pos1 = s_pos[pi];
        if (rid1 == rid0) valid = false;
      }
      uint32_t slot = NONE, v = 0;
      const uint64_t pair = rid0 < rid1 ? ((uint64_t)rid0 << 32 | rid1) : ((uint64_t)rid1 << 32 | rid0);
      if (valid) slot = pair_find(r, pair, &v);
      bool present = false, accepted = false, guessed = false;
      uint32_t ptype = 0, type = 0, mslot = NONE;
      if (valid) {
        present = v != 0 && own_bucket(v) < j;
        ptype = present ? own_type(v) : 0;
        if (!present && dup) {
          for (uint32_t i = (uint32_t)mix64(pair) & (SET_CAP - 1);; i = (i + 1) & (SET_CAP - 1)) {
            const unsigned long long kk = s_setk[i];
            if (kk == 0) break;
            if (kk == pair + 1) {
              present = true, ptype = s_sett[i];
              break;
            }
          }
        }
        if (!present) {
          const uint32_t rlen1 = s_rl[pi], dir1 = s_dir[pi];
          const uint32_t q_off = pos0 - pos1;
          if (q_off >= (1u << 30)) atomicOr(&r.c->overflow, OV_QOFF);
          uint32_t req = NONE;
          if (r.memo_used) mslot = memo_find(r, (unsigned long long)rid0 << 32 | rid1, q_off << 2 | dir0 << 1 | dir1, &req);
          if (req < r.settled) {
            accepted = classify(r.rq_res[req], rlen0, rlen1, q_off, &type);
          } else {
            accepted = true, guessed = true, type = T_OVERLAP;
            if (r.predict && predict_contained(rlen0, rlen1, q_off, r.predict, r.predict2)) type = rlen0 >= rlen1 ? T_CONTAINS : T_CONTAINED;
          }
        }
      }
      resolve_pending();
      const bool ins0 = valid && !present && accepted;
      uint32_t my_claim = NONE;
      if (dup) {
        if (ins0) {
          for (uint32_t i = (uint32_t)(mix64(pair) >> 20) & (CLAIM_CAP - 1);; i = (i + 1) & (CLAIM_CAP - 1)) {
            unsigned long long kk = s_clk[i];
            if (kk == 0) kk = atomicCAS(&s_clk[i], 0ULL, (unsigned long long)pair + 1), kk = kk ? kk : pair + 1;
            if (kk == pair + 1) {
              atomicMin(&s_clw[i], wi);
              my_claim = i;
              break;
            }
          }
        }
      }
      {
        const uint64_t mv = __ballot(valid), mp = __ballot(valid && present), mpo = __ballot(valid && present && ptype == T_OVERLAP);
        const uint64_t ma = __ballot(ins0), mao = __ballot(ins0 && type == T_OVERLAP), mac = __ballot(ins0 && type == T_CONTAINED);
        const uint64_t map = __ballot(ins0 && type == T_CONTAINS), mgu = __ballot(ins0 && guessed), muf = __ballot(ins0 && mslot == NONE);
        if (lane == 0)
          s_m[w][MV] = mv, s_m[w][MP] = mp, s_m[w][MPO] = mpo, s_m[w][MA] = ma, s_m[w][MAO] = mao, s_m[w][MAC] = mac, s_m[w][MAP] = map,
          s_m[w][MGU] = mgu, s_m[w][MUF] = muf, s_m[w][MDF] = 0;
      }
      __syncthreads();
      if (dup) {
        bool dflag = false;
        if (my_claim != NONE) {
          dflag = s_clw[my_claim] < wi;
        } else if (valid && !present) {
          for (uint32_t i = (uint32_t)(mix64(pair) >> 20) & (CLAIM_CAP - 1);; i = (i + 1) & (CLAIM_CAP - 1)) {
            const unsigned long long kk = s_clk[i];
            if (kk == 0) break;
            if (kk == pair + 1) {
              dflag = s_clw[i] < wi;
              break;
            }
          }
        }
        const uint64_t mdf = __ballot(dflag);
        if (lane == 0) s_m[w][MDF] = mdf;
        __syncthreads();
      }
      if (s_abort) break;
      M128 proc[BIG_NR];
#pragma unroll
      for (int k = 0; k < BIG_NR; ++k) proc[k] = M128{0, 0};
      int committed = 0;
      bool open_next = false;
      int open_row = 0;
      uint32_t open_pbase = 0, open_got = 0;
      for (int k = 0; k < nrows; ++k) {
        const uint32_t first_k = row_open ? pbase : (uint32_t)(a[k] + 1);
        const M128 gone = shr128(M128{clo, chi}, first_k);
        const M128 inc = andn128(M128{s_m[2 * k][MPO] | s_m[2 * k][MAO], s_m[2 * k + 1][MPO] | s_m[2 * k + 1][MAO]}, gone);
        const M128 ac = andn128(M128{s_m[2 * k][MAC], s_m[2 * k + 1][MAC]}, gone), ap = andn128(M128{s_m[2 * k][MAP], s_m[2 * k + 1][MAP]}, gone);
        const M128 df = andn128(M128{s_m[2 * k][MDF], s_m[2 * k + 1][MDF]}, gone);
        const int cut = any128(df) ? ctz128(df) : 128;
        if (cut == 0) break;
        const uint32_t need = r.bestn - (row_open ? got : 0u);
        int stop = 128;
        if ((uint32_t)popc128(inc) >= need) stop = nth128(inc, need);
        if (any128(ac)) stop = min(stop, ctz128(ac));
        const bool complete = stop < cut || (cut == 128);
        proc[k] = andn128(complete ? upto128(stop) : upto128(cut - 1), gone);
        const M128 apk = and128(ap, proc[k]);
        for (uint64_t m = apk.lo; m; m &= m - 1) cset(first_k + (uint32_t)__builtin_ctzll(m));
        for (uint64_t m = apk.hi; m; m &= m - 1) cset(first_k + 64u + (uint32_t)__builtin_ctzll(m));
        const bool rowc = any128(and128(ac, proc[k]));
        if (rowc) cset((uint32_t)a[k]);
        if (!complete) {
          open_next = true, open_row = a[k], open_pbase = first_k + (uint32_t)cut, open_got = (row_open ? got : 0u) + (uint32_t)popc128(and128(inc, proc[k]));
          break;
        }
        ++committed;
      }
#ifdef PGX_BIG_STATS
      ++st_steps, st_rows += (uint32_t)committed, st_cut += open_next ? 1u : 0u, st_full += (committed == nrows) ? 1u : 0u;
      st_cont += (!open_next && committed < nrows) ? 1u : 0u;
#endif
      if (committed) done_to = a[committed - 1];
      row_open = open_next;
      if (open_next) cur_row = open_row, pbase = open_pbase, got = open_got;
      uint32_t cins = 0, before = 0;
      uint64_t myproc = 0;
      for (int ww = 0; ww < BIG_NW; ++ww) {
        const int k = ww >> 1;
        const uint64_t pw = (ww & 1) ? proc[k].hi : proc[k].lo;
        const uint32_t c = (uint32_t)__popcll(s_m[ww][MA] & pw);
        if (ww < w) before += c;
        if (ww == w) myproc = pw;
        cins += c;
        skips += (uint32_t)__popcll(s_m[ww][MP] & pw);
        lookups += (uint32_t)__popcll(s_m[ww][MV] & ~s_m[ww][MP] & pw);
        any_guess |= (s_m[ww][MGU] & pw) != 0, any_unfiled |= (s_m[ww][MUF] & pw) != 0;
      }
      const uint32_t cur_no = num ? (num - 1) >> 4 : 0, first_new = num ? cur_no + 1 : 0;
      const uint32_t last = num + cins - 1, last_no = last >> 4;
      const uint32_t nnew = cins && last_no + 1 > first_new ? last_no + 1 - first_new : 0;
      if (threadIdx.x == 0 && nnew) {
        const uint32_t want = 16u * nnew;
        if (icur + want > iend) {
          const uint32_t take = want > ICH ? want : ICH;
          const uint32_t base = atomicAdd(&r.c->item_top, take);
          if ((uint64_t)base + take > r.item_cap) atomicOr(&r.c->overflow, OV_ITEMS), s_abort = 1;
          icur = base, iend = base + take;
        }
        s_fresh = icur, icur += want;
      }
      const bool visited = valid && ((myproc >> lane) & 1);
      {
        bool reg = visited;
        if (reg && slot == NONE) slot = pair_slot(r, pair);
        if (reg && !first_eval) {
          const uint32_t *pw = reinterpret_cast<const uint32_t *>(&r.pc[slot >> r.cshift]);
          const uint4 h1 = *reinterpret_cast<const uint4 *>(pw);
          const uint32_t c = min(h1.x, NIN);
          if ((c > 0 && h1.z == j + 1) || (c > 1 && h1.w == j + 1)) reg = false;
          for (uint32_t qq = 2; qq < c && reg; qq += 8) {
            const uint4 xa = *reinterpret_cast<const uint4 *>(pw + 2 + qq), xb = *reinterpret_cast<const uint4 *>(pw + 6 + qq);
            const uint32_t x[8] = {xa.x, xa.y, xa.z, xa.w, xb.x, xb.y, xb.z, xb.w};
#pragma unroll
            for (uint32_t k = 0; k < 8; ++k)
              if (qq + k < c && x[k] == j + 1) reg = false;
          }
        }
        if (reg) p_idx = atomicAdd(&r.pc[slot >> r.cshift].cnt, 1u), p_slot = slot, p_reg = true;
      }
      const bool my_ins = ins0 && visited;
      if (dup) {
        if (my_claim != NONE) s_clk[my_claim] = 0, s_clw[my_claim] = 0xFFFFFFFFu;
        if (my_ins) {
          uint32_t tries = 0;
          for (uint32_t i = (uint32_t)mix64(pair) & (SET_CAP - 1);; i = (i + 1) & (SET_CAP - 1)) {
            const unsigned long long kk = atomicCAS(&s_setk[i], 0ULL, (unsigned long long)pair + 1);
            if (kk == 0 || kk == pair + 1) {
              s_sett[i] = (uint8_t)type;
              break;
            }
            if (++tries >= SET_CAP) {
              s_bail = 1;
              break;
            }
          }
        }
      }
      __syncthreads();
      if (s_abort) break;
      if (cins) {
        const uint32_t fresh = s_fresh;
        auto base_of = [&](uint32_t no) { return no >= first_new ? fresh + 16u * (no - first_new) : chunk; };
        if (my_ins) {
          const uint32_t ord = num + before + (uint32_t)__popcll(s_m[w][MA] & myproc & ((1ULL << lane) - 1ULL));
          const uint32_t idx = base_of(ord >> 4) + (ord & 15);
          uint32_t next;
          if (ord == 0) next = NIL;
          else if ((ord & 15) == 0) next = base_of((ord >> 4) - 1) + 16;
          else next = idx;
          uint32_t info = (uint32_t)myrow | pi << 8 | type << 16;
          if (guessed) info |= I_GUESS;
          if (mslot == NONE) info |= I_UNFILED;
          r.items[idx] = Item{slot, info, mslot, next};
        }
        chunk = base_of(last_no);
        head = chunk + (last & 15) + 1;
        num += cins;
      }
      __syncthreads();
      if (s_bail) break;
    }
    resolve_pending();
#ifdef PGX_BIG_STATS
    if (threadIdx.x == 0) {
      unsigned long long *line = r.spread + (blockIdx.x % SPREAD) * 8;
      atomicAdd(line + 3, (unsigned long long)st_steps), atomicAdd(line + 4, (unsigned long long)st_rows), atomicAdd(line + 5, (unsigned long long)st_cut);
      atomicAdd(line + 6, (unsigned long long)st_cont), atomicAdd(line + 7, (unsigned long long)st_full);
      atomicMax(&r.c->big_max_steps, st_steps);
      if (st_steps >= 64) atomicAdd(&r.c->big_long, 1u), atomicAdd(&r.c->big_long_n, n);
      atomicAdd(&r.c->big_evals, 1u);
    }
#endif
    if (threadIdx.x == 0) {
      if (s_bail) {
        r.dirty[j] = 1, r.evaluated[j] = 0, r.parity[j] ^= 1;
        r.bflags[j] = (uint8_t)((r.bflags[j] & ~F_BIG));
      } else {
        r.ihead[j] = head, r.inum[j] = num, r.lookups[j] = lookups, r.skips[j] = skips;
        r.bflags[j] = (uint8_t)(F_BIG | (dup ? F_DUP : 0) | (any_guess ? F_GUESS : 0) | (any_unfiled ? F_UNFILED : 0));
      }
    }
  }
  if (s_abort) break;
  }
  if (lane == 0) r.wcur[wave_id] = make_uint4(rcur, rend, icur, iend);
}

}
}
```

peregrine_amd/csrc/pgx_replay_tables.hip:

```cpp
#include "pgx_replay.h"

namespace pgx {
namespace rp {

__global__ __launch_bounds__(256) void k_setup(R r, uint32_t *hist) {
  const uint32_t j = blockIdx.x * blockDim.x + threadIdx.x;
  if (j >= r.nb) return;
  const uint32_t b = r.bid[j], s0 = r.bstart[b], n = r.bstart[b + 1] - s0;
  bool dup = false;
  for (uint32_t i = 0; i + 1 < n && !dup; ++i) {
    const uint32_t ri = (uint32_t)(r.y0[s0 + i] >> 32);
    for (uint32_t k = i + 1; k < n; ++k)
      if ((uint32_t)(r.y0[s0 + k] >> 32) == ri) {
        dup = true;
        break;
      }
  }
  const bool big = dup ? r.dup_min && n >= r.dup_min : r.big_min && n >= r.big_min;
  r.bflags[j] = (uint8_t)((dup ? F_DUP : 0) | (big ? F_BIG : 0));
  if (big) atomicAdd(&r.c->nbig_total, 1u);
  r.dirty[j] = 1;
  if (hist) atomicAdd(&hist[(dup ? 16 : 0) + min(n / 8, 15u)], 1u);
}

__global__ void k_init_slots(uint4 *__restrict__ wcur, uint32_t nslots, uint32_t n_dense, uint32_t wlist0, Counters *c) {
  const uint32_t w = blockIdx.x * blockDim.x + threadIdx.x;
  if (w == 0) c->item_top = (n_dense + (nslots - wlist0)) * ICH;
  if (w >= nslots) return;
  if (w < n_dense || w >= wlist0) {
    const uint32_t piece = w < n_dense ? w : n_dense + (w - wlist0);
    wcur[w] = make_uint4(0u, 0u, piece * ICH, (piece + 1) * ICH);
  } else {
    wcur[w] = make_uint4(0u, 0u, 0u, 0u);
  }
}

__device__ __forceinline__ void apply_insertion(const R &r, uint32_t j, uint32_t pnew, const Item &im) {
  const uint32_t slot = im.pslot, type = (im.info >> 16) & 3;
  const uint32_t mine = own_enc(j, pnew, type);
  uint32_t v = r.ph[slot].own;
  for (;;) {
    if (v != 0 && own_bucket(v) < j) {
      r.dirty[j] = 1;
      return;
    }
    const uint32_t prev = atomicCAS(&r.ph[slot].own, v, mine);
    if (prev == v) {
      if (v == 0 || own_bucket(v) > j) mark_readers(r, slot, j);
      else if ((own_type(v) == T_OVERLAP) != (type == T_OVERLAP)) mark_readers(r, slot, j);
      return;
    }
    v = prev;
  }
}
__global__ __launch_bounds__(256) void k_update(R r, uint32_t lo, uint32_t hi, uint32_t nlist) {
  const int lane = threadIdx.x & 63, gl = lane & (GL - 1);
  const uint32_t wave = (blockIdx.x * blockDim.x + threadIdx.x) >> 6;
  const uint64_t jj = bucket_of_group(r, lo, hi, nlist, wave * GPW + (uint32_t)(lane / GL)) & 0x7FFFFFFFull;
  const uint32_t j = (uint32_t)jj;
  const bool alive = jj < hi && r.evaluated[j] && !r.c->overflow;
  if (blockIdx.x == 0 && threadIdx.x == 0) r.c->nbig = 0;
  if (!__ballot(alive)) return;
  const uint32_t pnew = alive ? r.parity[j] : 0, pold = pnew ^ 1;
  uint32_t cur = alive ? r.ihead[j] : NIL;
  while (__ballot(cur != NIL)) {
    if (cur != NIL) {
      const uint32_t last = cur - 1, base = last & ~15u, cnt = (last & 15) + 1;
      const Item first = r.items[base];
      for (uint32_t o = (uint32_t)gl; o < cnt; o += GL) apply_insertion(r, j, pnew, o == 0 ? first : r.items[base + o]);
      cur = first.next;
    }
  }
  cur = alive ? r.ohead[j] : NIL;
  while (__ballot(cur != NIL)) {
    if (cur != NIL) {
      const uint32_t last = cur - 1, base = last & ~15u, cnt = (last & 15) + 1;
      const uint32_t nxt = r.items[base].next;
      for (uint32_t o = (uint32_t)gl; o < cnt; o += GL) {
        const uint32_t slot = r.items[base + o].pslot;
        const uint32_t v = r.ph[slot].own;
        if (v != 0 && own_bucket(v) == j && own_parity(v) == pold)
          if (atomicCAS(&r.ph[slot].own, v, 0u) == v) mark_readers(r, slot, j);
      }
      cur = nxt;
    }
  }
  if (alive && gl == 0) r.evaluated[j] = 0, r.ohead[j] = NIL;
}

__device__ __forceinline__ uint32_t dirty16(const R &r, uint32_t j0, uint32_t end) {
  if (j0 >= end) return 0;
  uint32_t m = 0;
  if (j0 + 16 <= end) {
    const uint4 v = *reinterpret_cast<const uint4 *>(r.dirty + j0);
    const uint32_t w[4] = {v.x, v.y, v.z, v.w};
#pragma unroll
    for (int q = 0; q < 4; ++q)
#pragma unroll
      for (int b = 0; b < 4; ++b) m |= ((w[q] >> (8 * b)) & 0xFFu) ? 1u << (4 * q + b) : 0u;
  } else {
    for (uint32_t i = 0; j0 + i < end; ++i) m |= r.dirty[j0 + i] ? 1u << i : 0u;
  }
  return m;
}
__global__ __launch_bounds__(256) void k_count_a(R r, uint32_t rlo, uint32_t rhi, uint32_t *__restrict__ blk) {
  __shared__ uint32_t s_c[4], s_lo[4], s_hi[4];
  const uint32_t j0 = rlo + blockIdx.x * CB + threadIdx.x * 16;
  const uint32_t m = dirty16(r, j0, rhi);
  uint32_t c = (uint32_t)__popc(m), lo = m ? j0 + (uint32_t)__builtin_ctz(m) : 0xFFFFFFFFu, hi = m ? j0 + 31u - (uint32_t)__builtin_clz(m) : 0u;
  for (int o = 32; o; o >>= 1) {
    c += (uint32_t)__shfl_xor((int)c, o, 64);
    lo = min(lo, (uint32_t)__shfl_xor((int)lo, o, 64));
    hi = max(hi, (uint32_t)__shfl_xor((int)hi, o, 64));
  }
  const int w = threadIdx.x >> 6;
  if ((threadIdx.x & 63) == 0) s_c[w] = c, s_lo[w] = lo, s_hi[w] = hi;
  __syncthreads();
  if (threadIdx.x == 0) {
    if (blockIdx.x == 0) r.c->nbig = 0;
    blk[3 * blockIdx.x] = s_c[0] + s_c[1] + s_c[2] + s_c[3];
    blk[3 * blockIdx.x + 1] = min(min(s_lo[0], s_lo[1]), min(s_lo[2], s_lo[3]));
    blk[3 * blockIdx.x + 2] = max(max(s_hi[0], s_hi[1]), max(s_hi[2], s_hi[3]));
  }
}
__global__ __launch_bounds__(256) void k_count_b(R r, uint32_t rlo, uint32_t rhi, const uint32_t *__restrict__ blk, uint32_t nblk) {
  __shared__ uint32_t s_part[4], s_lo[4], s_hi[4], s_tot[4], s_w[4];
  uint32_t before = 0, total = 0, lo = 0xFFFFFFFFu, hi = 0;
  const bool totals = blockIdx.x == 0;
  for (uint32_t b = threadIdx.x; b < nblk; b += 256) {
    const uint32_t c = blk[3 * b];
    if (b < blockIdx.x) before += c;
    if (totals) total += c, lo = min(lo, blk[3 * b + 1]), hi = max(hi, blk[3 * b + 2]);
  }
  for (int o = 32; o; o >>= 1) {
    before += (uint32_t)__shfl_xor((int)before, o, 64);
    if (totals) {
      total += (uint32_t)__shfl_xor((int)total, o, 64);
      lo = min(lo, (uint32_t)__shfl_xor((int)lo, o, 64));
      hi = max(hi, (uint32_t)__shfl_xor((int)hi, o, 64));
    }
  }
  const int w = threadIdx.x >> 6, lane = threadIdx.x & 63;
  if (lane == 0) s_part[w] = before, s_tot[w] = total, s_lo[w] = lo, s_hi[w] = hi;
  const uint32_t j0 = rlo + blockIdx.x * CB + threadIdx.x * 16;
  const uint32_t m = dirty16(r, j0, rhi);
  const uint32_t c = (uint32_t)__popc(m);
  uint32_t incl = c;
  for (int o = 1; o < 64; o <<= 1) {
    const uint32_t t = (uint32_t)__shfl_up((int)incl, o, 64);
    if (lane >= o) incl += t;
  }
  if (lane == 63) s_w[w] = incl;
  __syncthreads();
  if (totals && threadIdx.x == 0) {
    const uint32_t n = s_tot[0] + s_tot[1] + s_tot[2] + s_tot[3];
    r.c->ndirty = n;
    r.c->min_dirty = n ? min(min(s_lo[0], s_lo[1]), min(s_lo[2], s_lo[3])) : 0xFFFFFFFFu;
    r.c->max_dirty = n ? max(max(s_hi[0], s_hi[1]), max(s_hi[2], s_hi[3])) : 0u;
  }
  if (!m) return;
  uint32_t at = s_part[0] + s_part[1] + s_part[2] + s_part[3] + incl - c;
  for (int q = 0; q < w; ++q) at += s_w[q];
  for (uint32_t mm = m; mm && at < LIST_CAP; mm &= mm - 1, ++at) {
    const uint32_t j = j0 + (uint32_t)__builtin_ctz(mm);
    const bool big = (r.bflags[j] & F_BIG) != 0;
    r.dlist[at] = j | (big ? 0x80000000u : 0u);
    if (big) {
      const uint32_t bat = atomicAdd(&r.c->nbig, 1u);
      if (bat < LIST_CAP) r.blist[bat] = at | 0x80000000u;
    }
  }
}

__device__ __forceinline__ void file_entries(const R &r, uint32_t s0, uint32_t row, uint32_t par) {
  const Ent e0 = entry_of(r.y0[s0 + row]), e1 = entry_of(r.y0[s0 + par]);
  if (e0.pos1 < e1.pos1 || e0.rid == e1.rid) return;
  const uint32_t dir0 = r.dir[s0 + row], dir1 = r.dir[s0 + par], q_off = e0.pos1 - e1.pos1;
  if (q_off >= (1u << 30)) return;
  const unsigned long long a = (unsigned long long)e0.rid << 32 | e1.rid;
  const uint32_t bk = q_off << 2 | dir0 << 1 | dir1;
  uint32_t i = (uint32_t)mix64(a ^ mix64(bk)) & r.mmask;
  for (int probes = 0; probes < 1024; ++probes) {
    unsigned long long cur = r.mt[i].a;
    if (cur == 0) {
      cur = atomicCAS(&r.mt[i].a, 0ULL, a);
      if (cur == 0) {
        r.mt[i].b = bk + 1;
        const uint32_t my = atomicAdd(&r.c->nreq, 1u);
        if (my >= r.req_cap) {
          atomicOr(&r.c->overflow, OV_REQS);
          return;
        }
        pgx_align_key key;
        key.rid0 = e0.rid, key.rid1 = e1.rid, key.q_off = q_off, key.dir0 = (uint8_t)dir0, key.dir1 = (uint8_t)dir1, key.pad[0] = key.pad[1] = 0;
        r.rq_key[my] = key;
        r.mt[i].req = my;
        return;
      }
    }
    if (cur == a && *(volatile uint32_t *)&r.mt[i].b == bk + 1) return;
    i = (i + 1) & r.mmask;
  }
}
__device__ __forceinline__ void file_for_reader(const R &r, uint32_t C, uint32_t rid_a, uint32_t rid_b) {
  const uint32_t b = r.bid[C], s0 = r.bstart[b], n = r.bstart[b + 1] - s0;
  int ia = -1, ib = -1;
  bool twice = false;
  for (uint32_t i = 0; i < n; ++i) {
    const uint32_t rid = (uint32_t)(r.y0[s0 + i] >> 32);
    if (rid == rid_a) twice |= ia >= 0, ia = (int)i;
    else if (rid == rid_b) twice |= ib >= 0, ib = (int)i;
  }
  if (ia < 0 || ib < 0 || twice) return;
  file_entries(r, s0, (uint32_t)min(ia, ib), (uint32_t)max(ia, ib));
}

__global__ __launch_bounds__(256) void k_file(R r, uint32_t limit) {
  const uint32_t j = blockIdx.x * blockDim.x + threadIdx.x;
  const bool active = j < limit && (r.bflags[j] & F_UNFILED) && !r.dirty[j];
  __shared__ uint32_t s_tot[4], s_base;
  if (!__syncthreads_or(active)) return;
  uint32_t cnt = 0;
  if (active)
    for (uint32_t it = r.ihead[j]; it != NIL; it = r.items[it - 1].next) cnt += (r.items[it - 1].info & I_UNFILED) ? 1u : 0u;
  const int lane = threadIdx.x & 63, wv = threadIdx.x >> 6;
  uint32_t incl = cnt;
  for (int o = 1; o < 64; o <<= 1) {
    const uint32_t t = (uint32_t)__shfl_up((int)incl, o, 64);
    if (lane >= o) incl += t;
  }
  const uint32_t total = (uint32_t)__shfl((int)incl, 63, 64);
  if (lane == 63) s_tot[wv] = total;
  __syncthreads();
  if (threadIdx.x == 0) {
    const uint32_t all = s_tot[0] + s_tot[1] + s_tot[2] + s_tot[3];
    s_base = all ? atomicAdd(&r.c->nreq, all) : 0u;
  }
  __syncthreads();
  uint32_t base = s_base;
  for (int w = 0; w < wv; ++w) base += s_tot[w];
  if (!__ballot(active)) return;
  bool run = active && cnt != 0;
  if (active && !cnt) r.bflags[j] &= (uint8_t)~F_UNFILED;
  if (!__ballot(run)) return;
  if ((unsigned long long)base + total > r.req_cap) {
    if (run) atomicOr(&r.c->overflow, OV_REQS);
    return;
  }
  uint32_t my = base + incl - cnt;
  const uint32_t b = run ? r.bid[j] : 0u, s0 = run ? r.bstart[b] : 0u;
  uint32_t it = run ? r.ihead[j] : NIL;
  const bool tail = r.tail != 0;
  const uint32_t nn = run ? r.bstart[b + 1] - s0 : 0u;
  for (;;) {
    bool fan = false;
    bool ah = false;
    uint32_t f_slot = 0, f_a = 0, f_b = 0, ah_ai = 0, ah_pi = 0;
    while (it != NIL && !fan && !ah) {
      Item &im = r.items[it - 1];
      const uint32_t nxt = im.next;
      if (im.info & I_UNFILED) {
        const uint32_t ai = im.info & 0xFF, pi = (im.info >> 8) & 0xFF;
        const Ent e0 = entry_of(r.y0[s0 + ai]), e1 = entry_of(r.y0[s0 + pi]);
        const uint32_t dir0 = r.dir[s0 + ai], dir1 = r.dir[s0 + pi], q_off = e0.pos1 - e1.pos1;
        const unsigned long long a = (unsigned long long)e0.rid << 32 | e1.rid;
        const uint32_t bk = q_off << 2 | dir0 << 1 | dir1;
        pgx_align_key key;
        key.rid0 = e0.rid, key.rid1 = e1.rid, key.q_off = q_off, key.dir0 = (uint8_t)dir0, key.dir1 = (uint8_t)dir1, key.pad[0] = key.pad[1] = 0;
        uint32_t i = (uint32_t)mix64(a ^ mix64(bk)) & r.mmask, found = NONE;
        bool fresh = false;
        for (int probes = 0; probes < 1024; ++probes) {
          unsigned long long cur = r.mt[i].a;
          if (cur == 0) {
            cur = atomicCAS(&r.mt[i].a, 0ULL, a);
            if (cur == 0) {
              r.mt[i].b = bk + 1;
              found = i, fresh = true;
              break;
            }
          }
          if (cur == a && *(volatile uint32_t *)&r.mt[i].b == bk + 1) {
            found = i;
            break;
          }
          i = (i + 1) & r.mmask;
        }
        if (found == NONE) {
          atomicOr(&r.c->overflow, OV_MEMO);
          run = false, it = NIL;
          break;
        }
        r.rq_key[my] = key;
        if (fresh) r.mt[found].req = my;
        ++my;
        im.mslot = found;
        im.info &= ~I_UNFILED;
        if (tail) ah = true, ah_ai = ai, ah_pi = pi;
        if (tail && fresh) fan = true, f_slot = im.pslot, f_a = e0.rid, f_b = e1.rid;
      }
      it = nxt;
    }
    const uint64_t fm = __ballot(fan), am = __ballot(ah);
    if (!fm && !am && !__ballot(it != NIL)) break;
    for (uint64_t mm = am; mm; mm &= mm - 1) {
      const int L = __builtin_ctzll(mm);
      const uint32_t sL = (uint32_t)__shfl((int)s0, L, 64), aL = (uint32_t)__shfl((int)ah_ai, L, 64), pL = (uint32_t)__shfl((int)ah_pi, L, 64);
      const uint32_t nL = (uint32_t)__shfl((int)nn, L, 64);
      for (uint32_t p = pL + 1 + (uint32_t)lane; p < nL && p <= pL + r.tail; p += 64) file_entries(r, sL, aL, p);
    }
    for (uint64_t mm = fm; mm; mm &= mm - 1) {
      const int L = __builtin_ctzll(mm);
      const uint32_t ps = (uint32_t)__shfl((int)f_slot, L, 64), ra = (uint32_t)__shfl((int)f_a, L, 64), rb2 = (uint32_t)__shfl((int)f_b, L, 64);
      const uint32_t jj = (uint32_t)__shfl((int)j, L, 64);
      const uint32_t *w = reinterpret_cast<const uint32_t *>(&r.pc[ps >> r.cshift]);
      const uint32_t c = min(w[0], NIN);
      for (uint32_t q = (uint32_t)lane; q < c; q += 64) {
        const uint32_t rb = w[2 + q];
        if (rb != 0 && rb - 1 != jj && rb - 1 < r.nb) file_for_reader(r, rb - 1, ra, rb2);
      }
      if (c >= NIN) {
        uint32_t idx = 0;
        for (uint32_t nd = w[1]; nd != NIL; nd = r.rn[nd - 1].next, ++idx)
          if ((idx & 63u) == (uint32_t)lane) {
            const uint32_t rb = r.rn[nd - 1].bucket;
            if (rb != jj && rb < r.nb) file_for_reader(r, rb, ra, rb2);
          }
      }
    }
  }
  if (run) r.bflags[j] &= (uint8_t)~F_UNFILED;
}

__global__ __launch_bounds__(256) void k_settle(R r) {
  const uint32_t j = blockIdx.x * blockDim.x + threadIdx.x;
  if (j >= r.nb || !(r.bflags[j] & F_GUESS)) return;
  const uint32_t b = r.bid[j], s0 = r.bstart[b];
  bool bad = false, remain = false;
  for (uint32_t it = r.ihead[j]; it != NIL; it = r.items[it - 1].next) {
    Item &im = r.items[it - 1];
    if (!(im.info & I_GUESS)) continue;
    const uint32_t req = im.mslot != NONE ? r.mt[im.mslot].req : NONE;
    if (req >= r.settled) {
      remain = true;
      continue;
    }
    const uint32_t ai = im.info & 0xFF, pi = (im.info >> 8) & 0xFF, gtype = (im.info >> 16) & 3;
    const Ent e0 = entry_of(r.y0[s0 + ai]), e1 = entry_of(r.y0[s0 + pi]);
    uint32_t type;
    const bool acc = classify(r.rq_res[req], r.rlen[e0.rid], r.rlen[e1.rid], e0.pos1 - e1.pos1, &type);
    if (!acc || type != gtype) bad = true;
#ifdef PGX_SETTLE_STATS
    if (!acc || type != gtype) {
      const uint32_t rl0 = r.rlen[e0.rid], rl1 = r.rlen[e1.rid], qo = e0.pos1 - e1.pos1;
      const uint32_t ol = min(rl0 - qo, rl1);
      const pgx_match mm = r.rq_res[req];
      int cat = acc ? 3 : (ol <= 520 ? 4 : (mm.q_end == 0 && mm.t_end == 0 ? 5 : 6));
      atomicAdd(&r.spread[((j >> 6) % SPREAD) * 8 + cat], 1ULL);
    }
#endif
    else im.info &= ~I_GUESS;
  }
  if (bad) r.dirty[j] = 1;
  if (!remain) r.bflags[j] &= (uint8_t)~F_GUESS;
}

__global__ __launch_bounds__(256) void k_emit(R r, const uint32_t *__restrict__ off, pgx_ovlp *__restrict__ out) {
  const uint32_t j = blockIdx.x * blockDim.x + threadIdx.x;
  unsigned long long lk = 0, sk = 0, ck = 0;
  if (j < r.nb) {
    lk = r.lookups[j], sk = r.skips[j];
    const uint32_t num = r.inum[j];
    if (num) {
      const uint32_t b = r.bid[j], s0 = r.bstart[b];
      uint32_t k = 0;
      for (uint32_t it = r.ihead[j]; it != NIL; it = r.items[it - 1].next, ++k) {
        const Item im = r.items[it - 1];
        const uint32_t ai = im.info & 0xFF, pi = (im.info >> 8) & 0xFF;
        const uint64_t ya = r.y0[s0 + ai], yb = r.y0[s0 + pi];
        pgx_ovlp o;
        o.y0 = ya, o.y1 = yb;
        o.rl0 = r.rlen[(uint32_t)(ya >> 32)], o.rl1 = r.rlen[(uint32_t)(yb >> 32)];
        o.strand0 = r.dir[s0 + ai], o.strand1 = r.dir[s0 + pi], o.ovlp_type = (uint8_t)((im.info >> 16) & 3), o.pad0 = 0;
        o.match = r.rq_res[r.mt[im.mslot].req];
        o.pad1 = 0;
        out[(size_t)off[j] + (num - 1 - k)] = o;
        ck += record_checksum(o, (uint64_t)off[j] + (num - 1 - k));
      }
    }
  }
  for (int o = 32; o; o >>= 1) {
    lk += (unsigned long long)__shfl_xor((int)(lk >> 32), o, 64) << 32 | (uint32_t)__shfl_xor((int)lk, o, 64);
    sk += (unsigned long long)__shfl_xor((int)(sk >> 32), o, 64) << 32 | (uint32_t)__shfl_xor((int)sk, o, 64);
    ck += (unsigned long long)__shfl_xor((int)(ck >> 32), o, 64) << 32 | (uint32_t)__shfl_xor((int)ck, o, 64);
  }
  if ((threadIdx.x & 63) == 0 && (lk | sk | ck)) {
    unsigned long long *line = r.spread + ((j >> 6) % SPREAD) * 8;
    atomicAdd(line + 1, lk);
    atomicAdd(line + 2, sk);
#if !defined(PGX_BIG_STATS) && !defined(PGX_SETTLE_STATS)
    atomicAdd(line + 7, ck);
#endif
  }
}

__global__ __launch_bounds__(256) void k_count_pairs(const PHot *__restrict__ ph, uint32_t cap, unsigned long long *__restrict__ out) {
  uint32_t c = 0;
  for (size_t i = (size_t)blockIdx.x * blockDim.x + threadIdx.x; i < cap; i += (size_t)gridDim.x * blockDim.x) c += ph[i].key != 0;
  for (int o = 32; o; o >>= 1) c += (uint32_t)__shfl_xor((int)c, o, 64);
  if ((threadIdx.x & 63) == 0 && c) atomicAdd(out, (unsigned long long)c);
}

}
}
```

Measured before the change: 62.86 million.

## Dispatch big buckets from a precomputed position list and add zoned dirty tracking

In dense passes, big buckets are no longer collected at run time by atomic appends inside the eval kernels. Instead a host-side sorted list of big-bucket positions is built once at setup, and each pass launches k_eval_big only over the big buckets in its range, or skips the launch when there are none. Separately, a zoned reader-entry encoding (zone bits in the top of the reader id, per-zone dirty bits via atomicOr) is added, but it is only enabled under PGX_BIG_STATS, so by default it compiles down to the old behaviour. The change removes atomic list building and empty big-kernel launches, at the cost of extra setup work, a host sync and a select pass.

```diff
diff --git a/peregrine_amd/csrc/pgx_replay.h b/peregrine_amd/csrc/pgx_replay.h
--- a/peregrine_amd/csrc/pgx_replay.h
+++ b/peregrine_amd/csrc/pgx_replay.h
@@ -46,6 +46,18 @@
 enum : uint32_t { OV_ITEMS = 1, OV_NODES = 2, OV_REQS = 4, OV_PAIRS = 8, OV_MEMO = 16, OV_QOFF = 32, OV_PASSES = 64 };
 constexpr uint8_t F_DUP = 1, F_GUESS = 2, F_UNFILED = 4;
 constexpr uint8_t F_BIG = 8;
+
+#ifdef PGX_BIG_STATS
+constexpr bool ZONED = true;
+#else
+constexpr bool ZONED = false;
+#endif
+constexpr uint32_t NZONE = 8, ENT_ZONE_AT = 29, ENT_ID = (1u << ENT_ZONE_AT) - 1u;
+constexpr uint8_t DIRTY_ALL = ZONED ? 0xFF : 1;
+__device__ __forceinline__ uint32_t ent_id(uint32_t e) { return ZONED ? e & ENT_ID : e; }
+__device__ __forceinline__ uint32_t ent_zone(uint32_t e) { return ZONED ? e >> ENT_ZONE_AT : 0u; }
+__device__ __forceinline__ uint32_t ent_enc(uint32_t id, uint32_t zone) { return ZONED ? id | zone << ENT_ZONE_AT : id; }
+__device__ __forceinline__ uint32_t zone_of(uint32_t row, uint32_t n) { return row * NZONE / n; }
 
 struct alignas(64) Counters {
   uint32_t item_top, rnode_top, nreq, overflow;
@@ -58,6 +70,7 @@
 #ifdef PGX_BIG_STATS
   uint32_t big_max_steps, big_long, big_long_n, big_evals;
   unsigned long long pad2[2];
+  unsigned long long z_evals, z_steps, z_skip, d_evals, d_steps, d_skip, pad3[2];
 #else
   unsigned long long pad2[4];
 #endif
@@ -87,6 +100,7 @@
   uint32_t *ihead, *inum, *ohead, *lookups, *skips;
   uint32_t *dlist;
   uint32_t *blist;
+  const uint32_t *bigpos;
   uint32_t wlist0;
   uint4 *wcur;
   Counters *c;
@@ -203,24 +217,53 @@
   return (uint64_t)lo + g;
 }
 
+__device__ __forceinline__ void dirty_mark(const R &r, uint32_t j, uint32_t zones) {
+  if (ZONED) atomicOr(reinterpret_cast<uint32_t *>(r.dirty + (j & ~3u)), zones << (8 * (j & 3u)));
+  else r.dirty[j] = 1;
+}
+
 __device__ __forceinline__ void mark_readers(const R &r, uint32_t slot, uint32_t j) {
   const uint32_t *w = reinterpret_cast<const uint32_t *>(&r.pc[slot >> r.cshift]);
   const uint4 h1 = *reinterpret_cast<const uint4 *>(w);
   const uint32_t c = min(h1.x, NIN);
-  if (c > 0 && h1.z > j + 1 && h1.z <= r.nb) r.dirty[h1.z - 1] = 1;
-  if (c > 1 && h1.w > j + 1 && h1.w <= r.nb) r.dirty[h1.w - 1] = 1;
+  auto mark = [&](uint32_t x) {
+    const uint32_t id = ent_id(x);
+    if (id > j + 1 && id <= r.nb) dirty_mark(r, id - 1, 1u << ent_zone(x));
+  };
+  if (c > 0) mark(h1.z);
+  if (c > 1) mark(h1.w);
   for (uint32_t q = 2; q < c; q += 8) {
     const uint4 a = *reinterpret_cast<const uint4 *>(w + 2 + q), b = *reinterpret_cast<const uint4 *>(w + 6 + q);
     const uint32_t x[8] = {a.x, a.y, a.z, a.w, b.x, b.y, b.z, b.w};
 #pragma unroll
     for (uint32_t k = 0; k < 8; ++k)
-      if (q + k < c && x[k] > j + 1 && x[k] <= r.nb) r.dirty[x[k] - 1] = 1;
+      if (q + k < c) mark(x[k]);
   }
   if (c < NIN) return;
   for (uint32_t nd = h1.y; nd != NIL; nd = r.rn[nd - 1].next) {
-    const uint32_t rb = r.rn[nd - 1].bucket;
-    if (rb > j) r.dirty[rb] = 1;
-  }
+    const uint32_t e = r.rn[nd - 1].bucket, rb = ent_id(e);
+    if (rb > j) dirty_mark(r, rb, 1u << ent_zone(e));
+  }
+}
+
+__device__ __forceinline__ bool reader_listed(uint32_t *w, const uint4 &h1, uint32_t c, uint32_t enc) {
+  const uint32_t id = ent_id(enc);
+  bool found = false;
+  auto look = [&](uint32_t x, uint32_t at) {
+    if (ent_id(x) != id) return;
+    found = true;
+    if (ZONED && x < enc) atomicMax(w + 2 + at, enc);
+  };
+  if (c > 0) look(h1.z, 0);
+  if (c > 1) look(h1.w, 1);
+  for (uint32_t q = 2; q < c && !found; q += 8) {
+    const uint4 a = *reinterpret_cast<const uint4 *>(w + 2 + q), b = *reinterpret_cast<const uint4 *>(w + 6 + q);
+    const uint32_t x[8] = {a.x, a.y, a.z, a.w, b.x, b.y, b.z, b.w};
+#pragma unroll
+    for (uint32_t k = 0; k < 8; ++k)
+      if (q + k < c) look(x[k], q + k);
+  }
+  return found;
 }
 
 struct M128 {
@@ -264,7 +307,7 @@
 constexpr uint32_t SET_CAP = 2048, CLAIM_CAP = 1024;
 constexpr uint32_t CB = 4096;
 
-__global__ void k_setup(R r, uint32_t *hist);
+__global__ void k_setup(R r, uint32_t *hist, uint8_t *is_big);
 __global__ void k_init_slots(uint4 *__restrict__ wcur, uint32_t nslots, uint32_t n_dense, uint32_t wlist0, Counters *c);
 __global__ void k_eval(R r, uint32_t lo, uint32_t hi, uint32_t nlist);
 template <int GLT, int PW>
diff --git a/peregrine_amd/csrc/pgx_replay.hip b/peregrine_amd/csrc/pgx_replay.hip
--- a/peregrine_amd/csrc/pgx_replay.hip
+++ b/peregrine_amd/csrc/pgx_replay.hip
@@ -1,3 +1,4 @@
+#include <algorithm>
 #include <optional>
 
 #include "pgx_replay.h"
@@ -144,7 +145,8 @@
   const int inner = env_int("PGX_REPLAY_K", 2);
   Sizes z;
   Tables tab;
-  DevBuf<uint32_t> bid, words, dlist, blist, cblk;
+  DevBuf<uint32_t> bid, words, dlist, blist, cblk, bigpos;
+  std::vector<uint32_t> h_bigpos;
   DevBuf<Item> items;
   DevBuf<RNode> rn;
   DevBuf<pgx_align_key> rq_key;
@@ -189,8 +191,9 @@
     alloc_tagged("replay.items", items, r.item_cap), alloc_tagged("replay.reader_nodes", rn, r.rn_cap);
     alloc_tagged("replay.requests", rq_key, r.req_cap), alloc_tagged("replay.requests", rq_res, r.req_cap);
     r.items = items.p, r.rn = rn.p, r.rq_key = rq_key.p, r.rq_res = rq_res.p;
-    bytes.alloc(nb * 5), words.alloc(nb * 5);
-    r.dirty = bytes.p, r.evaluated = bytes.p + nb, r.parity = bytes.p + 2 * nb, r.bflags = bytes.p + 3 * nb, r.ever = bytes.p + 4 * nb;
+    const size_t nbs = (nb + 15) & ~(size_t)15;
+    bytes.alloc(nbs * 5), words.alloc(nb * 5);
+    r.dirty = bytes.p, r.evaluated = bytes.p + nbs, r.parity = bytes.p + 2 * nbs, r.bflags = bytes.p + 3 * nbs, r.ever = bytes.p + 4 * nbs;
     r.ihead = words.p, r.inum = words.p + nb, r.ohead = words.p + 2 * nb, r.lookups = words.p + 3 * nb, r.skips = words.p + 4 * nb;
     wcur.alloc(nb + 2 + SPARSE_CAP + 1 + (size_t)BIG_WG * BIG_NW);
     r.wcur = wcur.p, r.wlist0 = (uint32_t)(nb + 2), r.wbig0 = (uint32_t)(nb + 2 + SPARSE_CAP + 1);
@@ -215,23 +218,33 @@
       const bool took = tab.hot_zero, took_cold = tab.cold_zero;
       tab.clear(s);
       if (trace && took) fprintf(stderr, "[pgx]   replay tables taken over pre-cleared (pair table%s, memo)\n", took_cold ? ", reader lists" : "");
-      PGX_HIP(hipMemsetAsync(bytes.p, 0, nb * 5, s));
+      PGX_HIP(hipMemsetAsync(bytes.p, 0, bytes.n, s));
       PGX_HIP(hipMemsetAsync(words.p, 0, nb * 5 * sizeof(uint32_t), s));
       PGX_HIP(hipMemsetAsync(dc.p, 0, sizeof(Counters), s));
       hipLaunchKernelGGL(k_init_slots, dim3(cdiv256(wcur.n)), dim3(256), 0, s, wcur.p, (uint32_t)wcur.n, (uint32_t)(nb / GPW + 2), r.wlist0, dc.p);
-      if (trace) setup_with_histogram();
-      else hipLaunchKernelGGL(k_setup, dim3(cdiv256(nb)), dim3(256), 0, s, r, (uint32_t *)nullptr);
-    }
-    if (r.big_min || r.dup_min) {
-      fetch(false);
-      use_big = hc->nbig_total != 0;
+      const bool may_big = r.big_min || r.dup_min;
+      DevBuf<uint8_t> is_big;
+      if (may_big) is_big.alloc(nb);
+      if (trace) setup_with_histogram(is_big.p);
+      else hipLaunchKernelGGL(k_setup, dim3(cdiv256(nb)), dim3(256), 0, s, r, (uint32_t *)nullptr, is_big.p);
+      if (may_big) {
+        fetch(false);
+        use_big = hc->nbig_total != 0;
+      }
+      if (use_big) {
+        alloc_tagged("replay.big_list", bigpos, hc->nbig_total);
+        h_bigpos.resize(select_indices(is_big.p, nb, bigpos.p));
+        bigpos.download(h_bigpos.data(), h_bigpos.size());
+        sync();
+        r.bigpos = bigpos.p;
+      }
     }
     cblk.alloc((nb + CB - 1) / CB * 3);
   }
-  void setup_with_histogram() {
+  void setup_with_histogram(uint8_t *is_big) {
     DevBuf<uint32_t> hist(32);
     PGX_HIP(hipMemsetAsync(hist.p, 0, 32 * sizeof(uint32_t), s));
-    hipLaunchKernelGGL(k_setup, dim3(cdiv256(nb)), dim3(256), 0, s, r, hist.p);
+    hipLaunchKernelGGL(k_setup, dim3(cdiv256(nb)), dim3(256), 0, s, r, hist.p, is_big);
     uint32_t h[32];
     hist.download(h, 32);
     sync();
@@ -257,6 +270,8 @@
     for (uint32_t i = 0; i < SPREAD; ++i) b3 += hs[i * 8 + 3], b4 += hs[i * 8 + 4], b5 += hs[i * 8 + 5], b6 += hs[i * 8 + 6], b7 += hs[i * 8 + 7];
     fprintf(stderr, "[pgx]   k_eval_big so far: %u evaluations, %llu steps, %llu rows committed; steps cut at a duplicate %llu, ended by a containment %llu, all rows %llu; longest %u steps, %u evaluations of >= 64 steps (entries %u)\n",
             hc->big_evals, b3, b4, b5, b6, b7, hc->big_max_steps, hc->big_long, hc->big_long_n);
+    fprintf(stderr, "[pgx]   k_eval_big re-evaluations so far: %llu of buckets without a repeated read, %llu steps, %llu of them in zones above the highest marked one; %llu of buckets with one, %llu steps, %llu above\n",
+            hc->z_evals, hc->z_steps, hc->z_skip, hc->d_evals, hc->d_steps, hc->d_skip);
 #endif
 #ifdef PGX_SETTLE_STATS
     unsigned long long c3 = 0, c4 = 0, c5 = 0, c6 = 0;
@@ -288,13 +303,19 @@
     if (walled) sync(), td = wall_ms();
     if (list == DEV_LIST_WIN) count(lo, hi);
     const uint32_t a = list ? 0u : lo, b = list ? (uint32_t)nb : hi;
-    const uint32_t big_a = list == DEV_LIST_WIN ? LIST_CAP : list == DEV_LIST ? groups : lo;
-    const dim3 big_grid(std::min<uint32_t>(BIG_WG, groups)), big_block(64 * BIG_NW), grid(cdiv256((size_t)groups * GL));
-    const bool side = use_big && list && !timed && !deep;
+    uint32_t big_a = list == DEV_LIST_WIN ? LIST_CAP : groups, big_b = b, big_n = groups;
+    if (!list && use_big) {
+      big_a = (uint32_t)(std::lower_bound(h_bigpos.begin(), h_bigpos.end(), lo) - h_bigpos.begin());
+      big_b = (uint32_t)(std::lower_bound(h_bigpos.begin(), h_bigpos.end(), hi) - h_bigpos.begin());
+      big_n = big_b - big_a;
+    }
+    const bool big = use_big && big_n != 0;
+    const dim3 big_grid(std::min<uint32_t>(BIG_WG, std::max(big_n, 1u))), big_block(64 * BIG_NW), grid(cdiv256((size_t)groups * GL));
+    const bool side = big && !timed && !deep;
     if (side) {
       PGX_HIP(hipEventRecord(rs.side_ev[0], s));
       PGX_HIP(hipStreamWaitEvent(rs.side_stream, rs.side_ev[0], 0));
-      hipLaunchKernelGGL(k_eval_big, big_grid, big_block, 0, rs.side_stream, r, big_a, b, list);
+      hipLaunchKernelGGL(k_eval_big, big_grid, big_block, 0, rs.side_stream, r, big_a, big_b, list);
       PGX_HIP(hipEventRecord(rs.side_ev[1], rs.side_stream));
     }
     if (narrow == Narrow::rows) hipLaunchKernelGGL((k_eval_rows<64, 16>), dim3(cdiv256((size_t)groups * 64)), dim3(256), 0, s, r, a, b, list);
@@ -302,9 +323,9 @@
     tm.reset();
     if (side) {
       PGX_HIP(hipStreamWaitEvent(s, rs.side_ev[1], 0));
-    } else if (use_big) {
+    } else if (big) {
       if (timed) tm.emplace("replay_big", 0);
-      hipLaunchKernelGGL(k_eval_big, big_grid, big_block, 0, s, r, big_a, b, list);
+      hipLaunchKernelGGL(k_eval_big, big_grid, big_block, 0, s, r, big_a, big_b, list);
       tm.reset();
     }
     if (walled) sync(), t_eval = wall_ms() - td, td = wall_ms();
diff --git a/peregrine_amd/csrc/pgx_replay_eval.hip b/peregrine_amd/csrc/pgx_replay_eval.hip
--- a/peregrine_amd/csrc/pgx_replay_eval.hip
+++ b/peregrine_amd/csrc/pgx_replay_eval.hip
@@ -11,13 +11,7 @@
   const uint64_t jj = bucket_of_group(r, lo, hi, nlist, wave * GPW + (uint32_t)(lane / GL));
   const uint32_t j = (uint32_t)jj;
   bool alive = jj < hi && r.dirty[j] && !r.c->overflow;
-  if (alive && (r.bflags[j] & F_BIG)) {
-    if (gl == 0) {
-      const uint32_t at = atomicAdd(&r.c->nbig, 1u);
-      if (at < LIST_CAP) r.blist[at] = j;
-    }
-    alive = false;
-  }
+  if (alive && (r.bflags[j] & F_BIG)) alive = false;
   {
     const uint64_t am = __ballot(alive);
     if (!am) return;
@@ -57,8 +51,9 @@
   uint32_t pbase = 0, got = 0, rid0 = 0, pos0 = 0, rlen0 = 0, dir0 = 0;
   bool p_reg = false;
   uint32_t p_idx = 0, p_slot = 0;
+  const uint32_t my_ent = ent_enc(j + 1, NZONE - 1);
   auto resolve_pending = [&]() -> bool {
-    if (p_reg && p_idx < NIN) r.pc[p_slot >> r.cshift].in[p_idx] = j + 1, p_reg = false;
+    if (p_reg && p_idx < NIN) r.pc[p_slot >> r.cshift].in[p_idx] = my_ent, p_reg = false;
     const uint64_t rm = __ballot(p_reg);
     if (rm) {
       const uint32_t total = (uint32_t)__popcll(rm);
@@ -75,7 +70,7 @@
       if (p_reg) {
         const uint32_t node = rcur + lane_rank(rm);
         const uint32_t old = atomicExch(&r.pc[p_slot >> r.cshift].rhead, node + 1);
-        r.rn[node] = RNode{old, j};
+        r.rn[node] = RNode{old, my_ent - 1};
       }
       rcur += total;
       p_reg = false;
@@ -164,17 +159,9 @@
       bool reg = valid && ((proc >> gl) & 1);
       if (reg && slot == NONE) slot = pair_slot(r, pair);
       if (reg && !first_eval) {
-        const uint32_t *w = reinterpret_cast<const uint32_t *>(&r.pc[slot >> r.cshift]);
+        uint32_t *w = reinterpret_cast<uint32_t *>(&r.pc[slot >> r.cshift]);
         const uint4 h1 = *reinterpret_cast<const uint4 *>(w);
-        const uint32_t c = min(h1.x, NIN);
-        if ((c > 0 && h1.z == j + 1) || (c > 1 && h1.w == j + 1)) reg = false;
-        for (uint32_t q = 2; q < c && reg; q += 8) {
-          const uint4 a = *reinterpret_cast<const uint4 *>(w + 2 + q), b = *reinterpret_cast<const uint4 *>(w + 6 + q);
-          const uint32_t x[8] = {a.x, a.y, a.z, a.w, b.x, b.y, b.z, b.w};
-#pragma unroll
-          for (uint32_t k = 0; k < 8; ++k)
-            if (q + k < c && x[k] == j + 1) reg = false;
-        }
+        if (reader_listed(w, h1, min(h1.x, NIN), my_ent)) reg = false;
       }
       if (reg) p_idx = atomicAdd(&r.pc[slot >> r.cshift].cnt, 1u), p_slot = slot, p_reg = true;
     }
@@ -259,13 +246,7 @@
   const uint64_t jj = bucket_of_group(r, lo, hi, nlist, wave * GPWT + (uint32_t)(lane / GLT));
   const uint32_t j = (uint32_t)jj;
   bool alive = jj < hi && r.dirty[j] && !r.c->overflow;
-  if (alive && (r.bflags[j] & F_BIG)) {
-    if (gl == 0) {
-      const uint32_t at = atomicAdd(&r.c->nbig, 1u);
-      if (at < LIST_CAP) r.blist[at] = j;
-    }
-    alive = false;
-  }
+  if (alive && (r.bflags[j] & F_BIG)) alive = false;
   {
     const uint64_t am = __ballot(alive);
     if (!am) return;
@@ -311,8 +292,9 @@
   uint32_t pbase = 0, got = 0;
   bool p_reg = false;
   uint32_t p_idx = 0, p_slot = 0;
+  const uint32_t my_ent = ent_enc(j + 1, NZONE - 1);
   auto resolve_pending = [&]() -> bool {
-    if (p_reg && p_idx < NIN) r.pc[p_slot >> r.cshift].in[p_idx] = j + 1, p_reg = false;
+    if (p_reg && p_idx < NIN) r.pc[p_slot >> r.cshift].in[p_idx] = my_ent, p_reg = false;
     const uint64_t rm = __ballot(p_reg);
     if (rm) {
       const uint32_t total = (uint32_t)__popcll(rm);
@@ -329,7 +311,7 @@
       if (p_reg) {
         const uint32_t node = rcur + lane_rank(rm);
         const uint32_t old = atomicExch(&r.pc[p_slot >> r.cshift].rhead, node + 1);
-        r.rn[node] = RNode{old, j};
+        r.rn[node] = RNode{old, my_ent - 1};
       }
       rcur += total;
       p_reg = false;
@@ -464,17 +446,9 @@
       bool reg = valid && ((proc >> gl) & 1);
       if (reg && slot == NONE) slot = pair_slot(r, pair);
       if (reg && !first_eval) {
-        const uint32_t *w = reinterpret_cast<const uint32_t *>(&r.pc[slot >> r.cshift]);
+        uint32_t *w = reinterpret_cast<uint32_t *>(&r.pc[slot >> r.cshift]);
         const uint4 h1 = *reinterpret_cast<const uint4 *>(w);
-        const uint32_t c = min(h1.x, NIN);
-        if ((c > 0 && h1.z == j + 1) || (c > 1 && h1.w == j + 1)) reg = false;
-        for (uint32_t qq = 2; qq < c && reg; qq += 8) {
-          const uint4 a = *reinterpret_cast<const uint4 *>(w + 2 + qq), b = *reinterpret_cast<const uint4 *>(w + 6 + qq);
-          const uint32_t x[8] = {a.x, a.y, a.z, a.w, b.x, b.y, b.z, b.w};
-#pragma unroll
-          for (uint32_t k = 0; k < 8; ++k)
-            if (qq + k < c && x[k] == j + 1) reg = false;
-        }
+        if (reader_listed(w, h1, min(h1.x, NIN), my_ent)) reg = false;
       }
       if (reg) p_idx = atomicAdd(&r.pc[slot >> r.cshift].cnt, 1u), p_slot = slot, p_reg = true;
     }
@@ -544,16 +518,21 @@
   uint32_t icur = wc.z, iend = wc.w;
   if (threadIdx.x == 0) s_abort = 0;
   const uint32_t list_limit = nlist ? lo : 0u;
-  const uint32_t nbig = min(r.c->nbig, LIST_CAP);
-  for (uint32_t g = blockIdx.x; g < nbig; g += gridDim.x) {
+  const uint32_t g_end = nlist ? min(r.c->nbig, LIST_CAP) : hi;
+  for (uint32_t g = (nlist ? 0u : lo) + blockIdx.x; g < g_end; g += gridDim.x) {
   {
-    const uint32_t e = r.blist[g];
-    if ((e & 0x80000000u) && (e & 0x7FFFFFFFu) >= list_limit) continue;
-    const uint32_t j = (e & 0x80000000u) ? (r.dlist[e & 0x7FFFFFFFu] & 0x7FFFFFFFu) : e;
+    uint32_t j;
+    if (nlist) {
+      const uint32_t e = r.blist[g] & 0x7FFFFFFFu;
+      if (e >= list_limit) continue;
+      j = r.dlist[e] & 0x7FFFFFFFu;
+    } else {
+      j = r.bigpos[g];
+    }
     __syncthreads();
     if (threadIdx.x == 0) {
       if (r.c->overflow) s_abort = 1;
-      s_bail = 0, s_fresh = (j < hi && r.dirty[j]) ? 1u : 0u;
+      s_bail = 0, s_fresh = (j < r.nb && r.dirty[j] && (r.bflags[j] & F_BIG)) ? 1u : 0u;
     }
     __syncthreads();
     if (s_abort) break;
@@ -561,6 +540,11 @@
     const uint32_t b = r.bid[j], s0 = r.bstart[b], n = r.bstart[b + 1] - s0;
     const bool first_eval = r.ever[j] == 0;
     const bool dup = (r.bflags[j] & F_DUP) != 0;
+    const bool zoned = ZONED;
+#ifdef PGX_BIG_STATS
+    const uint32_t marked = r.dirty[j];
+    const uint32_t top_zone = 31u - (uint32_t)__clz((int)(marked | 1u));
+#endif
     for (uint32_t i = threadIdx.x; i < n; i += blockDim.x) {
       const uint64_t y = r.y0[s0 + i];
       const uint32_t rid = (uint32_t)(y >> 32);
@@ -588,9 +572,9 @@
     int cur_row = 0;
     uint32_t pbase = 0, got = 0;
     bool p_reg = false;
-    uint32_t p_idx = 0, p_slot = 0;
+    uint32_t p_idx = 0, p_slot = 0, p_ent = 0;
     auto resolve_pending = [&]() {
-      if (p_reg && p_idx < NIN) r.pc[p_slot >> r.cshift].in[p_idx] = j + 1, p_reg = false;
+      if (p_reg && p_idx < NIN) r.pc[p_slot >> r.cshift].in[p_idx] = ZONED ? p_ent : j + 1, p_reg = false;
       const uint64_t rm = __ballot(p_reg);
       if (rm) {
         const uint32_t total = (uint32_t)__popcll(rm);
@@ -609,14 +593,14 @@
         if (p_reg) {
           const uint32_t node = rcur + lane_rank(rm);
           const uint32_t old = atomicExch(&r.pc[p_slot >> r.cshift].rhead, node + 1);
-          r.rn[node] = RNode{old, j};
+          r.rn[node] = RNode{old, ZONED ? p_ent - 1 : j};
         }
         rcur += total;
         p_reg = false;
       }
     };
 #ifdef PGX_BIG_STATS
-    uint32_t st_steps = 0, st_rows = 0, st_cut = 0, st_cont = 0, st_full = 0;
+    uint32_t st_steps = 0, st_rows = 0, st_cut = 0, st_cont = 0, st_full = 0, st_above = 0;
 #endif
     for (;;) {
       int a[BIG_NR], nrows = 0;
@@ -629,10 +613,14 @@
           do --x;
           while (x >= 0 && cget((uint32_t)x));
           if (x < 0) break;
+          if (zoned && nrows && zone_of((uint32_t)x, n) != zone_of((uint32_t)a[0], n)) break;
           a[nrows++] = x;
         }
       }
       if (nrows == 0 || r.bestn == 0) break;
+#ifdef PGX_BIG_STATS
+      st_above += zoned && zone_of((uint32_t)a[0], n) > top_zone ? 1u : 0u;
+#endif
       const int q = w >> 1, off = (w & 1) * 64 + lane;
       const int myrow = a[q];
       const uint32_t first = row_open ? pbase : (uint32_t)(myrow + 1);
@@ -790,20 +778,13 @@
       {
         bool reg = visited;
         if (reg && slot == NONE) slot = pair_slot(r, pair);
+        const uint32_t ent = ent_enc(j + 1, zoned ? zone_of((uint32_t)myrow, n) : NZONE - 1);
         if (reg && !first_eval) {
-          const uint32_t *pw = reinterpret_cast<const uint32_t *>(&r.pc[slot >> r.cshift]);
+          uint32_t *pw = reinterpret_cast<uint32_t *>(&r.pc[slot >> r.cshift]);
           const uint4 h1 = *reinterpret_cast<const uint4 *>(pw);
-          const uint32_t c = min(h1.x, NIN);
-          if ((c > 0 && h1.z == j + 1) || (c > 1 && h1.w == j + 1)) reg = false;
-          for (uint32_t qq = 2; qq < c && reg; qq += 8) {
-            const uint4 xa = *reinterpret_cast<const uint4 *>(pw + 2 + qq), xb = *reinterpret_cast<const uint4 *>(pw + 6 + qq);
-            const uint32_t x[8] = {xa.x, xa.y, xa.z, xa.w, xb.x, xb.y, xb.z, xb.w};
-#pragma unroll
-            for (uint32_t k = 0; k < 8; ++k)
-              if (qq + k < c && x[k] == j + 1) reg = false;
-          }
-        }
-        if (reg) p_idx = atomicAdd(&r.pc[slot >> r.cshift].cnt, 1u), p_slot = slot, p_reg = true;
+          if (reader_listed(pw, h1, min(h1.x, NIN), ent)) reg = false;
+        }
+        if (reg) p_idx = atomicAdd(&r.pc[slot >> r.cshift].cnt, 1u), p_slot = slot, p_ent = ent, p_reg = true;
       }
       const bool my_ins = ins0 && visited;
       if (dup) {
@@ -856,11 +837,14 @@
       atomicMax(&r.c->big_max_steps, st_steps);
       if (st_steps >= 64) atomicAdd(&r.c->big_long, 1u), atomicAdd(&r.c->big_long_n, n);
       atomicAdd(&r.c->big_evals, 1u);
+      if (!first_eval && !dup) atomicAdd(&r.c->z_evals, 1ULL), atomicAdd(&r.c->z_steps, (unsigned long long)st_steps), atomicAdd(&r.c->z_skip, (unsigned long long)st_above);
+      if (!first_eval && dup) atomicAdd(&r.c->d_evals, 1ULL), atomicAdd(&r.c->d_steps, (unsigned long long)st_steps), atomicAdd(&r.c->d_skip, (unsigned long long)st_above);
     }
 #endif
     if (threadIdx.x == 0) {
       if (s_bail) {
-        r.dirty[j] = 1, r.evaluated[j] = 0, r.parity[j] ^= 1;
+        r.dirty[j] = DIRTY_ALL, r.evaluated[j] = 0, r.parity[j] ^= 1;
+        __threadfence();
         r.bflags[j] = (uint8_t)((r.bflags[j] & ~F_BIG));
       } else {
         r.ihead[j] = head, r.inum[j] = num, r.lookups[j] = lookups, r.skips[j] = skips;
diff --git a/peregrine_amd/csrc/pgx_replay_tables.hip b/peregrine_amd/csrc/pgx_replay_tables.hip
--- a/peregrine_amd/csrc/pgx_replay_tables.hip
+++ b/peregrine_amd/csrc/pgx_replay_tables.hip
@@ -3,7 +3,7 @@
 namespace pgx {
 namespace rp {
 
-__global__ __launch_bounds__(256) void k_setup(R r, uint32_t *hist) {
+__global__ __launch_bounds__(256) void k_setup(R r, uint32_t *hist, uint8_t *is_big) {
   const uint32_t j = blockIdx.x * blockDim.x + threadIdx.x;
   if (j >= r.nb) return;
   const uint32_t b = r.bid[j], s0 = r.bstart[b], n = r.bstart[b + 1] - s0;
@@ -19,7 +19,8 @@
   const bool big = dup ? r.dup_min && n >= r.dup_min : r.big_min && n >= r.big_min;
   r.bflags[j] = (uint8_t)((dup ? F_DUP : 0) | (big ? F_BIG : 0));
   if (big) atomicAdd(&r.c->nbig_total, 1u);
-  r.dirty[j] = 1;
+  if (is_big) is_big[j] = big ? 1 : 0;
+  r.dirty[j] = DIRTY_ALL;
   if (hist) atomicAdd(&hist[(dup ? 16 : 0) + min(n / 8, 15u)], 1u);
 }
 
@@ -35,13 +36,18 @@
   }
 }
 
+__device__ __forceinline__ uint32_t item_zone_mark(const R &r, uint32_t j, const Item &im) {
+  if (!ZONED) return 1u;
+  const uint32_t b = r.bid[j];
+  return 1u << zone_of(im.info & 0xFF, r.bstart[b + 1] - r.bstart[b]);
+}
 __device__ __forceinline__ void apply_insertion(const R &r, uint32_t j, uint32_t pnew, const Item &im) {
   const uint32_t slot = im.pslot, type = (im.info >> 16) & 3;
   const uint32_t mine = own_enc(j, pnew, type);
   uint32_t v = r.ph[slot].own;
   for (;;) {
     if (v != 0 && own_bucket(v) < j) {
-      r.dirty[j] = 1;
+      dirty_mark(r, j, item_zone_mark(r, j, im));
       return;
     }
     const uint32_t prev = atomicCAS(&r.ph[slot].own, v, mine);
@@ -315,14 +321,14 @@
       const uint32_t *w = reinterpret_cast<const uint32_t *>(&r.pc[ps >> r.cshift]);
       const uint32_t c = min(w[0], NIN);
       for (uint32_t q = (uint32_t)lane; q < c; q += 64) {
-        const uint32_t rb = w[2 + q];
+        const uint32_t rb = ent_id(w[2 + q]);
         if (rb != 0 && rb - 1 != jj && rb - 1 < r.nb) file_for_reader(r, rb - 1, ra, rb2);
       }
       if (c >= NIN) {
         uint32_t idx = 0;
         for (uint32_t nd = w[1]; nd != NIL; nd = r.rn[nd - 1].next, ++idx)
           if ((idx & 63u) == (uint32_t)lane) {
-            const uint32_t rb = r.rn[nd - 1].bucket;
+            const uint32_t rb = ent_id(r.rn[nd - 1].bucket);
             if (rb != jj && rb < r.nb) file_for_reader(r, rb, ra, rb2);
           }
       }
@@ -335,7 +341,8 @@
   const uint32_t j = blockIdx.x * blockDim.x + threadIdx.x;
   if (j >= r.nb || !(r.bflags[j] & F_GUESS)) return;
   const uint32_t b = r.bid[j], s0 = r.bstart[b];
-  bool bad = false, remain = false;
+  bool remain = false;
+  uint32_t bad = 0;
   for (uint32_t it = r.ihead[j]; it != NIL; it = r.items[it - 1].next) {
     Item &im = r.items[it - 1];
     if (!(im.info & I_GUESS)) continue;
@@ -348,7 +355,7 @@
     const Ent e0 = entry_of(r.y0[s0 + ai]), e1 = entry_of(r.y0[s0 + pi]);
     uint32_t type;
     const bool acc = classify(r.rq_res[req], r.rlen[e0.rid], r.rlen[e1.rid], e0.pos1 - e1.pos1, &type);
-    if (!acc || type != gtype) bad = true;
+    if (!acc || type != gtype) bad |= item_zone_mark(r, j, im);
 #ifdef PGX_SETTLE_STATS
     if (!acc || type != gtype) {
       const uint32_t rl0 = r.rlen[e0.rid], rl1 = r.rlen[e1.rid], qo = e0.pos1 - e1.pos1;
@@ -360,7 +367,7 @@
 #endif
     else im.info &= ~I_GUESS;
   }
-  if (bad) r.dirty[j] = 1;
+  if (bad) dirty_mark(r, j, bad);
   if (!remain) r.bflags[j] &= (uint8_t)~F_GUESS;
 }
 
```

Result: no change. 63.06 million (median of 6 runs) (+0.3%).
